# naver/dust3r

Hardware: NVIDIA H100
Metric: image-pairs/sec (512x384, ViT-L/B+DPT) (higher is better)
Workload: dtype bf16

## Files before the change

dust3r_b200/_lib_fwd.py:

```python
import ctypes as C

F_BIAS, F_GELU, F_RELU, F_OUT_F32, F_RESID_INPLACE = 1, 2, 4, 8, 16
F_ADD0, F_ADD1, F_OUT2_RELU, F_ROPE, F_OUT2_BF16 = 32, 64, 128, 256, 2048


class Linear(C.Structure):
    _fields_ = [('w', C.c_void_p), ('b', C.c_void_p)]


class Norm(C.Structure):
    _fields_ = [('g', C.c_void_p), ('b', C.c_void_p)]


class EncBlock(C.Structure):
    _fields_ = [('norm1', Norm), ('norm2', Norm), ('qkv', Linear), ('proj', Linear), ('fc1', Linear), ('fc2', Linear)]


class DecBlock(C.Structure):
    _fields_ = [('norm1', Norm), ('norm2', Norm), ('norm3', Norm), ('norm_y', Norm),
                ('qkv', Linear), ('proj', Linear), ('projq', Linear), ('projkv', Linear), ('cproj', Linear),
                ('fc1', Linear), ('fc2', Linear)]


class Fusion(C.Structure):
    _fields_ = [('rcu1_conv1', Linear), ('rcu1_conv2', Linear), ('rcu2_conv1', Linear), ('rcu2_conv2', Linear),
                ('out_conv', Linear)]


class DptHead(C.Structure):
    _fields_ = [('act_conv', Linear * 4), ('act0_up', Linear), ('act1_up', Linear), ('act3_down', Linear),
                ('layer_rn', Linear * 4), ('refine', Fusion * 4), ('head0', Linear), ('head2', Linear),
                ('head4_w', C.c_void_p), ('head4_b', C.c_void_p)]


class Model(C.Structure):
    _fields_ = [('enc_dim', C.c_int32), ('enc_depth', C.c_int32), ('enc_heads', C.c_int32), ('dec_dim', C.c_int32),
                ('dec_depth', C.c_int32), ('dec_heads', C.c_int32), ('mlp_ratio', C.c_int32), ('patch', C.c_int32),
                ('head_type', C.c_int32), ('nch', C.c_int32), ('depth_mode', C.c_int32), ('conf_mode', C.c_int32),
                ('conf_min', C.c_float), ('conf_max', C.c_float), ('ln_eps', C.c_float),
                ('hooks', C.c_int32 * 4), ('rope_max_pos', C.c_int32),
                ('rope_cos', C.c_void_p), ('rope_sin', C.c_void_p),
                ('patch_embed', Linear), ('enc', C.POINTER(EncBlock)), ('enc_norm', Norm), ('decoder_embed', Linear),
                ('dec1', C.POINTER(DecBlock)), ('dec2', C.POINTER(DecBlock)), ('dec_norm', Norm),
                ('dpt', C.POINTER(DptHead) * 2), ('lin_head', Linear * 2)]


def declare(lib):
    vp, i32, i64, u32, f32 = C.c_void_p, C.c_int32, C.c_int64, C.c_uint32, C.c_float
    lib.d3r_gemm_bf16.restype = C.c_int
    lib.d3r_gemm_bf16.argtypes = [vp, vp, vp, vp, vp, vp, i32, i32, i32, i64, u32, vp, vp, i32, i32, i32, vp]
    lib.d3r_conv3x3_bf16.restype = C.c_int
    lib.d3r_conv3x3_bf16.argtypes = [vp, vp, vp, vp, vp, vp, vp, i32, i32, i32, i32, i32, u32, vp]
    lib.d3r_attention_hd64.restype = C.c_int
    lib.d3r_attention_hd64.argtypes = [vp, i64, vp, i64, vp, i64, vp, i64, i32, i32, i32, i32, f32, vp]
    lib.d3r_conv_transpose_bf16.restype = C.c_int
    lib.d3r_conv_transpose_bf16.argtypes = [vp, vp, vp, vp, i32, i32, i32, i32, i32, i32, vp]
    lib.d3r_conv3x3_head_tail.restype = C.c_int
    lib.d3r_conv3x3_head_tail.argtypes = [vp, vp, vp, vp, vp, vp, vp, i32, i32, i32, i32, i32, f32, f32, vp]
    lib.d3r_layernorm_bf16.restype = C.c_int
    lib.d3r_layernorm_bf16.argtypes = [vp, vp, vp, vp, i32, i32, f32, vp]
    lib.d3r_upsample2x_bf16.restype = C.c_int
    lib.d3r_upsample2x_bf16.argtypes = [vp, vp, i32, i32, i32, i32, i32, i32, vp]
    lib.d3r_im2col_3x3_s2_bf16.restype = C.c_int
    lib.d3r_im2col_3x3_s2_bf16.argtypes = [vp, vp, i32, i32, i32, i32, vp]
    lib.d3r_patch_im2col16.restype = C.c_int
    lib.d3r_patch_im2col16.argtypes = [vp, vp, i32, i32, i32, vp]
    lib.d3r_linear_head_postprocess.restype = C.c_int
    lib.d3r_linear_head_postprocess.argtypes = [vp, vp, vp, i32, i32, i32, i32, i32, i32, f32, f32, vp]
    lib.d3r_set_gemm_impl.restype = None
    lib.d3r_set_gemm_impl.argtypes = [i32]
    lib.d3r_set_gemm_store.restype = None
    lib.d3r_set_gemm_store.argtypes = [i32]
    lib.d3r_set_attention_impl.restype = None
    lib.d3r_set_attention_impl.argtypes = [i32]
    lib.d3r_forward_workspace_bytes.restype = i64
    lib.d3r_forward_workspace_bytes.argtypes = [C.POINTER(Model), i32, i32, i32, i32]
    lib.d3r_forward_pairs.restype = C.c_int
    lib.d3r_forward_pairs.argtypes = [C.POINTER(Model), vp, i32, C.POINTER(i32), C.POINTER(i32), i32, i32, i32,
                                      vp, vp, vp, vp, vp, i64, vp]
    lib.d3r_forward_mixed_workspace_bytes.restype = i64
    lib.d3r_forward_mixed_workspace_bytes.argtypes = [C.POINTER(Model), i32, i32, i32, i32, i32]
    lib.d3r_forward_pairs_mixed.restype = C.c_int
    lib.d3r_forward_pairs_mixed.argtypes = [C.POINTER(Model), vp, i32, i32, vp, i32, i32, i32, vp, vp, vp, vp, vp, i64, vp]
    lib.d3r_forward_set_debug.restype = C.c_int
    lib.d3r_forward_set_debug.argtypes = [i32, vp, i64]
    lib.d3r_sizeof_model.restype = C.c_int
```

dust3r_b200/csrc/gemm_host.cu:

```cuda
#include "gemm_wgmma.cuh"
#include "gemm_host.h"
#include "prof.h"

namespace d3r {
namespace gemm {

static int pick_block_n(int N, int mode, uint32_t flags) {
  if (flags & F_HEAD_FINAL) return 128;
  if (N % 256 == 0 && pick_epi(mode, flags) != EPI_GENERIC) return 256;
  if (N % 128 == 0) return 128;
  if (N % 64 == 0) return 64;
  return (N > 128) ? 128 : 64;
}

static int g_impl = 2;
static int g_pair_min_kb = 4;
static bool use_pair(int bn, int num_kb) { return bn >= 128 && (g_impl == 1 || (g_impl == 2 && num_kb >= g_pair_min_kb)); }

static int g_store = 1;

template <int BN, int EPI, bool PAIR, bool TMA_STORE = false>
static int launch(const CUtensorMap& ta, const CUtensorMap& tb, const CUtensorMap& to, const Params& p, int m_tiles, int n_tiles,
                  cudaStream_t st) {
  constexpr int kSmem = Cfg<BN, TMA_STORE>::kSmemBytes;
  static unsigned long long attr_devices = 0;
  if (first_launch_on_this_device(attr_devices))
    D3R_CUDA(cudaFuncSetAttribute(gemm_kernel<BN, EPI, PAIR, TMA_STORE>, cudaFuncAttributeMaxDynamicSharedMemorySize, kSmem));
  int grid;
  if (PAIR) {
    const int items = ((m_tiles + 1) / 2) * n_tiles;
    const int max_clusters = num_sms() / 2;
    grid = 2 * (items < max_clusters ? items : max_clusters);
  } else {
    const int items = m_tiles * n_tiles;
    grid = items < num_sms() ? items : num_sms();
  }
  const char* tag = (p.mode == 1) ? ((p.flags & F_HEAD_FINAL) ? (PAIR ? "conv3x3_head_tail_2cta" : "conv3x3_head_tail")
                                                              : (PAIR ? "conv3x3_wgmma_2cta" : "conv3x3_wgmma"))
                                  : (BN == 256 ? (PAIR ? "gemm_wgmma_2cta_bn256" : "gemm_wgmma_bn256")
                                               : (PAIR ? "gemm_wgmma_2cta_bn128" : (BN == 128 ? "gemm_wgmma_bn128" : "gemm_wgmma_bn64")));
  char detail[96];
  snprintf(detail, sizeof(detail), "M=%d N=%d K=%d flags=0x%x mode=%d epi=%d", p.M, p.N, p.K, (unsigned)p.flags, p.mode, EPI);
  prof::Scope scope(tag, st, 2.0 * double(p.M) * double(p.N) * double(p.K), 0.0, 1, detail);
  D3R_CUDA(pdl::launch_clustered(gemm_kernel<BN, EPI, PAIR, TMA_STORE>, dim3(grid), dim3(kNumThreads), size_t(kSmem), st, PAIR ? 2 : 1,
                                 ta, tb, to, p));
  D3R_LAUNCH_CHECK();
  return D3R_OK;
}

template <int BN, bool PAIR>
static int dispatch_epi(int epi, const CUtensorMap& ta, const CUtensorMap& tb, const CUtensorMap* to, const Params& p, int m_tiles,
                        int n_tiles, cudaStream_t st) {
  if constexpr (BN == 256) {
    if (to) {
      switch (epi) {
        case EPI_RESID: return launch<BN, EPI_RESID, PAIR, true>(ta, tb, *to, p, m_tiles, n_tiles, st);
        case EPI_ACT: return launch<BN, EPI_ACT, PAIR, true>(ta, tb, *to, p, m_tiles, n_tiles, st);
        case EPI_ROPE: return launch<BN, EPI_ROPE, PAIR, true>(ta, tb, *to, p, m_tiles, n_tiles, st);
      }
    }
  }
  switch (epi) {
    case EPI_RESID: return launch<BN, EPI_RESID, PAIR>(ta, tb, tb, p, m_tiles, n_tiles, st);
    case EPI_ACT: return launch<BN, EPI_ACT, PAIR>(ta, tb, tb, p, m_tiles, n_tiles, st);
    case EPI_ROPE: return launch<BN, EPI_ROPE, PAIR>(ta, tb, tb, p, m_tiles, n_tiles, st);
  }
  if constexpr (BN == 128) return launch<128, EPI_GENERIC, PAIR>(ta, tb, tb, p, m_tiles, n_tiles, st);
  set_error("no BLOCK_N %d kernel for the generic epilogue", BN);
  return D3R_ERR_INVALID;
}

static int dispatch(int bn, const CUtensorMap& ta, const CUtensorMap& tb, const CUtensorMap* to, const Params& p, int m_tiles,
                    cudaStream_t st) {
  const int n_tiles = (p.N + bn - 1) / bn;
  const int epi = (bn >= 128) ? pick_epi(p.mode, p.flags) : EPI_GENERIC;
  const bool pair = use_pair(bn, p.num_kb);
  switch (bn) {
    case 256: return pair ? dispatch_epi<256, true>(epi, ta, tb, to, p, m_tiles, n_tiles, st) : dispatch_epi<256, false>(epi, ta, tb, to, p, m_tiles, n_tiles, st);
    case 128: return pair ? dispatch_epi<128, true>(epi, ta, tb, nullptr, p, m_tiles, n_tiles, st) : dispatch_epi<128, false>(epi, ta, tb, nullptr, p, m_tiles, n_tiles, st);
    case 64: return launch<64, EPI_GENERIC, false>(ta, tb, tb, p, m_tiles, n_tiles, st);
  }
  set_error("unsupported BLOCK_N %d", bn);
  return D3R_ERR_INVALID;
}

static int make_tmap_b(CUtensorMap* m, const void* B, int N, int taps, int Kc, int bn, int num_kb, const char* op) {
  cuuint64_t dims[3] = {(cuuint64_t)Kc, (cuuint64_t)taps, (cuuint64_t)N};
  cuuint64_t str[2] = {(cuuint64_t)Kc * 2, (cuuint64_t)taps * Kc * 2};
  cuuint32_t box[3] = {(cuuint32_t)BLOCK_K, 1, (cuuint32_t)(use_pair(bn, num_kb) ? bn / 2 : bn)};
  return encode_tensor_map(m, B, 3, dims, str, box, op);
}

int gemm_bf16(const void* A, long long lda, const void* B, Params p, cudaStream_t st) {
  D3R_CHECK_ARG(A && B, "gemm: null operand");
  D3R_CHECK_ARG(p.M > 0 && p.N > 0 && p.K > 0, "gemm: bad shape %d %d %d", p.M, p.N, p.K);
  D3R_CHECK_ARG(p.N % 32 == 0, "gemm: N=%d must be a multiple of 32", p.N);
  D3R_CHECK_ARG(p.K % 8 == 0 && lda % 8 == 0, "gemm: K=%d / lda=%lld must be multiples of 8 (16-byte TMA strides)", p.K, lda);
  D3R_CHECK_ARG((reinterpret_cast<uintptr_t>(A) & 15) == 0 && (reinterpret_cast<uintptr_t>(B) & 15) == 0, "gemm: operands must be 16-byte aligned");
  p.mode = 0;
  p.num_kb = (p.K + BLOCK_K - 1) / BLOCK_K;
  const int bn = pick_block_n(p.N, p.mode, p.flags);
  CUtensorMap ta, tb;
  {
    cuuint64_t dims[2] = {(cuuint64_t)p.K, (cuuint64_t)p.M};
    cuuint64_t str[1] = {(cuuint64_t)lda * 2};
    cuuint32_t box[2] = {(cuuint32_t)BLOCK_K, (cuuint32_t)BLOCK_M};
    int rc = encode_tensor_map(&ta, A, 2, dims, str, box, "gemm");
    if (rc) return rc;
  }
  int rc = make_tmap_b(&tb, B, p.N, 1, p.K, bn, p.num_kb, "gemm");
  if (rc) return rc;
  CUtensorMap to;
  const bool f32 = (p.flags & F_RESID_INPLACE) != 0;
  const long long row_bytes = p.ldo * (f32 ? 4 : 2);
  const bool staged = g_store == 1 && bn == 256 && pick_epi(p.mode, p.flags) != EPI_GENERIC && p.ldo >= p.N && row_bytes % 16 == 0 &&
                      (reinterpret_cast<uintptr_t>(p.out) & 15) == 0;
  if (staged) {
    cuuint64_t dims[2] = {(cuuint64_t)p.N, (cuuint64_t)p.M};
    cuuint64_t str[1] = {(cuuint64_t)row_bytes};
    cuuint32_t box[2] = {(cuuint32_t)(f32 ? 32 : 64), 64};
    rc = encode_tensor_map(&to, p.out, 2, dims, str, box, "gemm output", f32 ? CU_TENSOR_MAP_DATA_TYPE_FLOAT32 : CU_TENSOR_MAP_DATA_TYPE_BFLOAT16);
    if (rc) return rc;
  }
  return dispatch(bn, ta, tb, staged ? &to : nullptr, p, (p.M + BLOCK_M - 1) / BLOCK_M, st);
}

int conv3x3_bf16(const void* x_nhwc, const void* w_packed, int B, int H, int W, int Cin, int Cout, Params p, cudaStream_t st) {
  D3R_CHECK_ARG(x_nhwc && w_packed, "conv3x3: null operand");
  D3R_CHECK_ARG(Cin % 8 == 0 && Cout % 32 == 0, "conv3x3: Cin=%d must be a multiple of 8 and Cout=%d of 32", Cin, Cout);
  p.mode = 1;
  p.M = B * H * W;
  p.N = Cout;
  p.cin_blocks = (Cin + BLOCK_K - 1) / BLOCK_K;
  p.K = 9 * Cin;
  p.num_kb = 9 * p.cin_blocks;
  p.cB = B; p.cH = H; p.cW = W;
  int tw = 16;
  while (tw < W && tw < 128) tw *= 2;
  p.tile_w = tw;
  p.tile_h = BLOCK_M / tw;
  p.tiles_x = (W + p.tile_w - 1) / p.tile_w;
  p.tiles_y = (H + p.tile_h - 1) / p.tile_h;
  p.ldo = Cout;
  const int bn = pick_block_n(p.N, p.mode, p.flags);
  CUtensorMap ta, tb;
  {
    cuuint64_t dims[4] = {(cuuint64_t)Cin, (cuuint64_t)W, (cuuint64_t)H, (cuuint64_t)B};
    cuuint64_t str[3] = {(cuuint64_t)Cin * 2, (cuuint64_t)W * Cin * 2, (cuuint64_t)H * W * Cin * 2};
    cuuint32_t box[4] = {(cuuint32_t)BLOCK_K, (cuuint32_t)p.tile_w, (cuuint32_t)p.tile_h, 1};
    int rc = encode_tensor_map(&ta, x_nhwc, 4, dims, str, box, "conv3x3");
    if (rc) return rc;
  }
  int rc = make_tmap_b(&tb, w_packed, Cout, 9, Cin, bn, p.num_kb, "conv3x3");
  if (rc) return rc;
  return dispatch(bn, ta, tb, nullptr, p, B * p.tiles_x * p.tiles_y, st);
}

int conv_transpose_bf16(const void* x_nhwc, const void* w_packed, void* out, const float* bias, int B, int h, int w, int Cin, int Cout,
                        int k, cudaStream_t st) {
  D3R_CHECK_ARG(x_nhwc && w_packed && out, "conv_transpose: null buffer");
  D3R_CHECK_ARG(B > 0 && h > 0 && w > 0 && Cin > 0 && Cout > 0 && k > 0, "conv_transpose: bad shape B=%d h=%d w=%d Cin=%d Cout=%d k=%d", B,
                h, w, Cin, Cout, k);
  D3R_CHECK_ARG(Cin % 8 == 0, "conv_transpose: Cin=%d must be a multiple of 8", Cin);
  D3R_CHECK_ARG(Cout % 2 == 0 && (k * k * Cout) % 32 == 0, "conv_transpose: Cout=%d must be even and k*k*Cout=%d a multiple of 32", Cout,
                k * k * Cout);
  Params p{};
  p.M = B * h * w; p.N = k * k * Cout; p.K = Cin;
  p.flags = F_CONVT | (bias ? F_BIAS : 0);
  p.out = out; p.bias = bias; p.ldo = 0;
  p.tk = k; p.th_in = h; p.tw_in = w; p.tCout = Cout;
  return gemm_bf16(x_nhwc, Cin, w_packed, p, st);
}

int conv3x3_head_tail(const void* x_nhwc, const void* w_packed, const float* bias, const float* w4, const float* b4, float* pts3d,
                      float* conf, int B, int H, int W, int depth_mode, int conf_mode, float conf_min, float conf_max, cudaStream_t st) {
  D3R_CHECK_ARG(x_nhwc && w_packed && w4 && b4 && pts3d, "conv3x3_head_tail: null buffer");
  D3R_CHECK_ARG(B > 0 && H > 0 && W > 0, "conv3x3_head_tail: bad shape B=%d H=%d W=%d", B, H, W);
  D3R_CHECK_ARG(depth_mode >= 0 && depth_mode <= 2, "conv3x3_head_tail: depth_mode %d out of range", depth_mode);
  D3R_CHECK_ARG(conf_mode >= 0 && conf_mode <= 2, "conv3x3_head_tail: conf_mode %d out of range", conf_mode);
  D3R_CHECK_ARG(conf_mode == 0 || conf, "conv3x3_head_tail: conf_mode %d without a conf buffer", conf_mode);
  Params p{};
  p.flags = F_HEAD_FINAL | (bias ? F_BIAS : 0);
  p.bias = bias;
  p.w4 = w4; p.b4 = b4;
  p.pts3d = pts3d; p.conf = conf;
  p.depth_mode = depth_mode; p.conf_mode = conf_mode;
  p.conf_min = conf_min; p.conf_max = conf_max;
  return conv3x3_bf16(x_nhwc, w_packed, B, H, W, 128, 128, p, st);
}

}
}

using namespace d3r;

extern "C" void d3r_set_gemm_impl(int32_t impl) { gemm::g_impl = impl; }
extern "C" void d3r_set_gemm_pair_min_kblocks(int32_t kb) { gemm::g_pair_min_kb = kb; }
extern "C" void d3r_set_gemm_store(int32_t store) { gemm::g_store = store; }

extern "C" int d3r_gemm_bf16(const void* A, const void* B, void* out, const float* bias, const void* add0, void* out2,
                             int32_t M, int32_t N, int32_t K, int64_t ldo, uint32_t flags, const float* rope_cos,
                             const float* rope_sin, int32_t rope_cols, int32_t tokens_per_img, int32_t grid_w, void* stream) {
  gemm::Params p{};
  p.M = M; p.N = N; p.K = K;
  p.flags = flags;
  p.out = out; p.out2 = out2; p.add0 = add0; p.bias = bias; p.ldo = ldo;
  p.rope_cos = rope_cos; p.rope_sin = rope_sin; p.rope_cols = rope_cols; p.tokens_per_img = tokens_per_img; p.grid_w = grid_w;
  D3R_CHECK_ARG(!(flags & gemm::F_BIAS) || bias, "gemm: F_BIAS without bias");
  D3R_CHECK_ARG(!(flags & gemm::F_ROPE) || (rope_cos && rope_sin && tokens_per_img > 0 && grid_w > 0), "gemm: F_ROPE without tables");
  D3R_CHECK_ARG(!(flags & (gemm::F_CONVT | gemm::F_HEAD_FINAL)),
                "gemm: F_CONVT / F_HEAD_FINAL have their own entry points, d3r_conv_transpose_bf16 / d3r_conv3x3_head_tail");
  return gemm::gemm_bf16(A, K, B, p, (cudaStream_t)stream);
}

extern "C" int d3r_conv3x3_bf16(const void* x_nhwc, const void* w_packed, void* out, const float* bias, const void* add0,
                                const void* add1, void* out2, int32_t B, int32_t H, int32_t W, int32_t Cin, int32_t Cout,
                                uint32_t flags, void* stream) {
  gemm::Params p{};
  p.flags = flags;
  p.out = out; p.out2 = out2; p.add0 = add0; p.add1 = add1; p.bias = bias;
  D3R_CHECK_ARG(!(flags & (gemm::F_CONVT | gemm::F_HEAD_FINAL | gemm::F_ROPE)), "conv3x3: unsupported flag");
  return gemm::conv3x3_bf16(x_nhwc, w_packed, B, H, W, Cin, Cout, p, (cudaStream_t)stream);
}

extern "C" int d3r_conv_transpose_bf16(const void* x_nhwc, const void* w_packed, void* out, const float* bias, int32_t B, int32_t h,
                                       int32_t w, int32_t Cin, int32_t Cout, int32_t k, void* stream) {
  return gemm::conv_transpose_bf16(x_nhwc, w_packed, out, bias, B, h, w, Cin, Cout, k, (cudaStream_t)stream);
}

extern "C" int d3r_conv3x3_head_tail(const void* x_nhwc, const void* w_packed, const float* bias, const float* w4, const float* b4,
                                     float* pts3d, float* conf, int32_t B, int32_t H, int32_t W, int32_t depth_mode, int32_t conf_mode,
                                     float conf_min, float conf_max, void* stream) {
  return gemm::conv3x3_head_tail(x_nhwc, w_packed, bias, w4, b4, pts3d, conf, B, H, W, depth_mode, conf_mode, conf_min, conf_max,
                                 (cudaStream_t)stream);
}
```

dust3r_b200/csrc/gemm_wgmma.cuh:

```cuda
#pragma once
#include "d3r_common.cuh"
#include "sm90_ptx.cuh"
#include "pdl.cuh"

namespace d3r {
namespace gemm {

constexpr int BLOCK_M = 128;
constexpr int BLOCK_K = 64;
constexpr int WGMMA_K = 16;
constexpr int kNumThreads = 384;
constexpr int kConsumerWarps = 8;

enum : uint32_t {
  F_BIAS = 1u << 0,
  F_GELU = 1u << 1,
  F_RELU = 1u << 2,
  F_OUT_F32 = 1u << 3,
  F_RESID_INPLACE = 1u << 4,
  F_ADD0 = 1u << 5,
  F_ADD1 = 1u << 6,
  F_OUT2_RELU = 1u << 7,
  F_ROPE = 1u << 8,
  F_CONVT = 1u << 9,
  F_HEAD_FINAL = 1u << 10,
  F_OUT2_BF16 = 1u << 11,
};

struct Params {
  int M, N, K;
  int num_kb;
  int mode;
  uint32_t flags;
  void* out;
  void* out2;
  const void* add0;
  const void* add1;
  const float* bias;
  long long ldo;
  const float* rope_cos;
  const float* rope_sin;
  int rope_cols, tokens_per_img, grid_w;
  int cB, cH, cW, cin_blocks, tile_w, tile_h, tiles_x, tiles_y;
  int tk, th_in, tw_in, tCout;
  const float* w4;
  const float* b4;
  float* pts3d;
  float* conf;
  int depth_mode;
  int conf_mode;
  float conf_min, conf_max;
};

enum : int { EPI_GENERIC = 0, EPI_RESID = 1, EPI_ACT = 2, EPI_ROPE = 3 };
template <int EPI> struct EpiMask { static constexpr uint32_t value = 0xFFFFFFFFu; };
template <> struct EpiMask<EPI_RESID> { static constexpr uint32_t value = F_BIAS | F_RESID_INPLACE; };
template <> struct EpiMask<EPI_ACT> { static constexpr uint32_t value = F_BIAS | F_GELU | F_RELU; };
template <> struct EpiMask<EPI_ROPE> { static constexpr uint32_t value = F_BIAS | F_ROPE; };
__host__ __device__ inline int pick_epi(int mode, uint32_t flags) {
  if (mode != 0) return EPI_GENERIC;
  if ((flags & ~F_BIAS) == F_RESID_INPLACE) return EPI_RESID;
  if ((flags & ~EpiMask<EPI_ACT>::value) == 0) return EPI_ACT;
  if ((flags & ~EpiMask<EPI_ROPE>::value) == 0) return EPI_ROPE;
  return EPI_GENERIC;
}

template <int BLOCK_N, bool TMA_STORE = false>
struct Cfg {
  static constexpr int kStageA = BLOCK_M * BLOCK_K * 2;
  static constexpr int kStageB = BLOCK_N * BLOCK_K * 2;
  static constexpr int kStages = (BLOCK_N == 256) ? 4 : (BLOCK_N == 128) ? 6 : 8;
  static constexpr int kRing = kStages * (kStageA + kStageB);
  static constexpr int kOutBuf = 64 * 128;
  static constexpr int kStaging = TMA_STORE ? 2 * 2 * kOutBuf : 0;
  static constexpr int kSmemBytes = kRing + kStaging + 1024  + 256  + (TMA_STORE ? 0 : (4 * 128 + 16) * 4) ;
  static_assert(kSmemBytes <= 227 * 1024, "shared memory of one CTA");
};

__device__ __forceinline__ float gelu_erf(float x) {
  constexpr float kU = 0.84932180028801904f;
  constexpr float kP = 0.3275911f * 0.70710678118654752f / kU;
  const float u = fabsf(x) * kU;
  const float t = ptx::rcp_approx(fmaf(kP, u, 1.f));
  float poly = fmaf(0.5f * 1.061405429f, t, 0.5f * -1.453152027f);
  poly = fmaf(poly, t, 0.5f * 1.421413741f);
  poly = fmaf(poly, t, 0.5f * -0.284496736f);
  poly = fmaf(poly, t, 0.5f * 0.254829592f);
  const float e = ptx::ex2_approx(-u * u);
  const float h = x * (poly * t * e);
  return fmaxf(x, 0.f) - fabsf(h);
}

template <int BLOCK_N, int EPI, bool PAIR, bool TMA_STORE>
__global__ void __launch_bounds__(kNumThreads, 1)
gemm_kernel(const __grid_constant__ CUtensorMap tmap_a, const __grid_constant__ CUtensorMap tmap_b,
            const __grid_constant__ CUtensorMap tmap_o, const Params p) {
  static_assert(!TMA_STORE || (BLOCK_N == 256 && EPI != EPI_GENERIC), "TMA-store epilogue: specialised epilogues on 128x256 tiles");
  using C = Cfg<BLOCK_N, TMA_STORE>;
  extern __shared__ uint8_t smem_raw[];
  uint8_t* smem = reinterpret_cast<uint8_t*>((reinterpret_cast<uintptr_t>(smem_raw) + 1023) & ~uintptr_t(1023));
  uint8_t* smem_a = smem;
  uint8_t* smem_b = smem + C::kStages * C::kStageA;
  uint8_t* smem_o = smem + C::kRing;
  uint64_t* bars = reinterpret_cast<uint64_t*>(smem + C::kRing + C::kStaging);
  uint64_t* full_bar = bars;
  uint64_t* empty_bar = bars + C::kStages;
  float* s_w4 = reinterpret_cast<float*>(reinterpret_cast<uint8_t*>(bars) + 256);

  const int warp = threadIdx.x >> 5, lane = threadIdx.x & 31;
  const uint32_t rank = PAIR ? ptx::cluster_ctarank() : 0u;
  const int n_tiles = (p.N + BLOCK_N - 1) / BLOCK_N;
  const int m_tiles = (p.mode == 1) ? p.cB * p.tiles_y * p.tiles_x : (p.M + BLOCK_M - 1) / BLOCK_M;
  const int m_groups = PAIR ? (m_tiles + 1) / 2 : m_tiles;
  const int total_items = m_groups * n_tiles;
  const int first_item = PAIR ? blockIdx.x / 2 : blockIdx.x;
  const int item_stride = PAIR ? gridDim.x / 2 : gridDim.x;

  if (threadIdx.x == 0) {
    ptx::prefetch_tmap(&tmap_a);
    ptx::prefetch_tmap(&tmap_b);
    if constexpr (TMA_STORE) ptx::prefetch_tmap(&tmap_o);
    for (int s = 0; s < C::kStages; ++s) {
      ptx::mbar_init(ptx::smem_u32(&full_bar[s]), 1);
      ptx::mbar_init(ptx::smem_u32(&empty_bar[s]), (PAIR ? 2 : 1) * kConsumerWarps);
    }
    ptx::fence_barrier_init();
  }
  if (!TMA_STORE && (p.flags & F_HEAD_FINAL) && threadIdx.x >= 128) {
    for (int i = threadIdx.x - 128; i < 4 * 128 + 4; i += 256) s_w4[i] = (i < 512) ? p.w4[i] : p.b4[i - 512];
  }
  __syncthreads();
  if constexpr (PAIR) ptx::cluster_sync();
  pdl::sync_with_predecessor();

  if (warp < 4) {
    ptx::setmaxnreg_dec<40>();
    if (warp == 0 && ptx::elect_one()) {
      int stage = 0;
      uint32_t phase = 0;
      for (int item = first_item; item < total_items; item += item_stride) {
        const int tn = item % n_tiles, tm = (item / n_tiles) * (PAIR ? 2 : 1) + int(rank);
        int cb = 0, cy0 = 0, cx0 = 0;
        if (p.mode == 1) {
          cb = tm / (p.tiles_y * p.tiles_x);
          const int r = tm - cb * (p.tiles_y * p.tiles_x);
          cy0 = (r / p.tiles_x) * p.tile_h;
          cx0 = (r % p.tiles_x) * p.tile_w;
        }
        for (int kb = 0; kb < p.num_kb; ++kb) {
          ptx::mbar_wait(ptx::smem_u32(&empty_bar[stage]), phase ^ 1);
          const uint32_t fb = ptx::smem_u32(&full_bar[stage]);
          ptx::mbar_arrive_expect_tx(fb, C::kStageA + C::kStageB);
          const uint32_t sa = ptx::smem_u32(smem_a + stage * C::kStageA);
          const uint32_t sb = ptx::smem_u32(smem_b + stage * C::kStageB);
          int ka, kt = 0;
          if (p.mode == 1) {
            const int tap = kb / p.cin_blocks, cblk = kb - tap * p.cin_blocks;
            const int dy = tap / 3, dx = tap - dy * 3;
            ptx::tma_load_4d(sa, &tmap_a, fb, cblk * BLOCK_K, cx0 + dx - 1, cy0 + dy - 1, cb);
            ka = cblk * BLOCK_K;
            kt = tap;
          } else {
            ptx::tma_load_2d(sa, &tmap_a, fb, kb * BLOCK_K, tm * BLOCK_M);
            ka = kb * BLOCK_K;
          }
          if constexpr (PAIR) {
            constexpr int kHalf = BLOCK_N / 2;
            ptx::tma_load_3d_mc(sb + rank * (kHalf * BLOCK_K * 2), &tmap_b, fb, ka, kt, tn * BLOCK_N + int(rank) * kHalf, 0x3);
          } else {
            ptx::tma_load_3d(sb, &tmap_b, fb, ka, kt, tn * BLOCK_N);
          }
          if (++stage == C::kStages) { stage = 0; phase ^= 1; }
        }
      }
    }
  } else {
    ptx::setmaxnreg_inc<232>();
    const int wg = (threadIdx.x >> 7) - 1;
    const int wq = warp & 3;
    const int q = lane & 3;
    const uint32_t flags = p.flags & EpiMask<EPI>::value;
    constexpr int kNB = BLOCK_N / 8;
    float acc[BLOCK_N / 2];
    int stage = 0;
    uint32_t phase = 0;
    uint32_t out_chunk = 0;
    auto release = [&](int s) {
      if (lane == 0) {
        if constexpr (PAIR) {
          ptx::mbar_arrive_cluster(ptx::smem_u32(&empty_bar[s]), 0);
          ptx::mbar_arrive_cluster(ptx::smem_u32(&empty_bar[s]), 1);
        } else {
          ptx::mbar_arrive(ptx::smem_u32(&empty_bar[s]));
        }
      }
    };
    for (int item = first_item; item < total_items; item += item_stride) {
      const int tn = item % n_tiles, tm = (item / n_tiles) * (PAIR ? 2 : 1) + int(rank);
      int prev = -1;
      for (int kb = 0; kb < p.num_kb; ++kb) {
        ptx::mbar_wait(ptx::smem_u32(&full_bar[stage]), phase);
        const uint64_t da = ptx::desc_kmajor_sw128(ptx::smem_u32(smem_a + stage * C::kStageA + wg * 64 * 128));
        const uint64_t db = ptx::desc_kmajor_sw128(ptx::smem_u32(smem_b + stage * C::kStageB));
        ptx::wgmma_fence();
#pragma unroll
        for (int k = 0; k < BLOCK_K / WGMMA_K; ++k) {
          if constexpr (BLOCK_N == 256) ptx::wgmma_m64n256k16_ss(acc, da + uint64_t(2 * k), db + uint64_t(2 * k), (kb | k) != 0 ? 1u : 0u);
          else if constexpr (BLOCK_N == 128) ptx::wgmma_m64n128k16_ss(acc, da + uint64_t(2 * k), db + uint64_t(2 * k), (kb | k) != 0 ? 1u : 0u);
          else ptx::wgmma_m64n64k16_ss(acc, da + uint64_t(2 * k), db + uint64_t(2 * k), (kb | k) != 0 ? 1u : 0u);
        }
        ptx::wgmma_commit();
        ptx::wgmma_wait<1>();
        if (prev >= 0) release(prev);
        prev = stage;
        if (++stage == C::kStages) { stage = 0; phase ^= 1; }
      }
      ptx::wgmma_wait<0>();
      ptx::reg_fence(acc);
      release(prev);

      bool valid[2];
      long long row_off[2];
      int tok[2] = {0, 0};
      long long pix[2] = {0, 0};
      int ct_b[2] = {0, 0}, ct_iy[2] = {0, 0}, ct_ix[2] = {0, 0};
#pragma unroll
      for (int h = 0; h < 2; ++h) {
        const int row_in_tile = wg * 64 + wq * 16 + (lane >> 2) + 8 * h;
        if (p.mode == 1) {
          const int cb = tm / (p.tiles_y * p.tiles_x);
          const int r = tm - cb * (p.tiles_y * p.tiles_x);
          const int y = (r / p.tiles_x) * p.tile_h + row_in_tile / p.tile_w;
          const int x = (r % p.tiles_x) * p.tile_w + row_in_tile % p.tile_w;
          valid[h] = (tm < m_tiles) && (y < p.cH) && (x < p.cW);
          pix[h] = (long long)(cb * p.cH + y) * p.cW + x;
          row_off[h] = pix[h] * p.ldo;
        } else {
          const int row = tm * BLOCK_M + row_in_tile;
          valid[h] = row < p.M;
          row_off[h] = (long long)row * p.ldo;
          if (flags & F_ROPE) tok[h] = row % p.tokens_per_img;
          if (flags & F_CONVT) {
            ct_b[h] = row / (p.th_in * p.tw_in);
            const int r = row - ct_b[h] * (p.th_in * p.tw_in);
            ct_iy[h] = r / p.tw_in;
            ct_ix[h] = r - ct_iy[h] * p.tw_in;
          }
        }
      }
      if (flags & (F_BIAS | F_GELU)) {
#pragma unroll
        for (int j = 0; j < kNB; ++j) {
          const int c = tn * BLOCK_N + 8 * j + 2 * q;
          float2 b = make_float2(0.f, 0.f);
          if ((flags & F_BIAS) && c < p.N) {
            if (flags & F_CONVT) b = make_float2(__ldg(p.bias + c % p.tCout), __ldg(p.bias + (c + 1) % p.tCout));
            else b = __ldg(reinterpret_cast<const float2*>(p.bias + c));
          }
#pragma unroll
          for (int h = 0; h < 2; ++h) {
            float& v0 = acc[4 * j + 2 * h];
            float& v1 = acc[4 * j + 2 * h + 1];
            v0 += b.x;
            v1 += b.y;
            if (flags & F_GELU) { v0 = gelu_erf(v0); v1 = gelu_erf(v1); }
          }
        }
      }
      if (flags & F_ROPE) {
#pragma unroll
        for (int cb = 0; cb < BLOCK_N / 32; ++cb) {
          const int col0 = tn * BLOCK_N + cb * 32;
          if (col0 >= p.rope_cols) continue;
#pragma unroll
          for (int h = 0; h < 2; ++h) {
            const int pos = ((col0 & 63) < 32) ? (tok[h] / p.grid_w) : (tok[h] % p.grid_w);
#pragma unroll
            for (int jj = 0; jj < 2; ++jj) {
              const int k = 8 * jj + 2 * q;
              const float2 cs = __ldg(reinterpret_cast<const float2*>(p.rope_cos + pos * 16 + k));
              const float2 sn = __ldg(reinterpret_cast<const float2*>(p.rope_sin + pos * 16 + k));
              const float cc[2] = {cs.x, cs.y}, ss[2] = {sn.x, sn.y};
#pragma unroll
              for (int e = 0; e < 2; ++e) {
                float& u = acc[(4 * cb + jj) * 4 + 2 * h + e];
                float& w = acc[(4 * cb + jj + 2) * 4 + 2 * h + e];
                const float u0 = u, w0 = w;
                u = u0 * cc[e] - w0 * ss[e];
                w = w0 * cc[e] + u0 * ss[e];
              }
            }
          }
        }
      }
      if constexpr (TMA_STORE) {
        constexpr bool kF32 = (EPI == EPI_RESID);
        constexpr int kChunkCols = kF32 ? 32 : 64;
        constexpr int kChunkNB = kChunkCols / 8;
        const bool issuer = (threadIdx.x & 127) == 0;
        const uint32_t sw = lane >> 2;
#pragma unroll
        for (int c = 0; c < BLOCK_N / kChunkCols; ++c) {
          const uint32_t buf = ptx::smem_u32(smem_o + (wg * 2 + (out_chunk & 1)) * C::kOutBuf);
#pragma unroll
          for (int j = 0; j < kChunkNB; ++j)
#pragma unroll
            for (int h = 0; h < 2; ++h) {
              const uint32_t row = wq * 16 + (lane >> 2) + 8 * h;
              float v0 = acc[4 * (c * kChunkNB + j) + 2 * h], v1 = acc[4 * (c * kChunkNB + j) + 2 * h + 1];
              if (flags & F_RELU) { v0 = fmaxf(v0, 0.f); v1 = fmaxf(v1, 0.f); }
              if constexpr (kF32) {
                ptx::st_shared_v2_f32(buf + row * 128 + (((2 * j + (q >> 1)) ^ sw) << 4) + (q & 1) * 8, v0, v1);
              } else {
                ptx::st_shared_b32(buf + row * 128 + ((j ^ sw) << 4) + q * 4, pack_bf16x2(v0, v1));
              }
            }
          ptx::fence_proxy_async();
          if (issuer) ptx::bulk_wait_group_read<0>();
          ptx::named_bar_sync(1 + wg, 128);
          if (issuer) {
            const int c0 = tn * BLOCK_N + c * kChunkCols, r0 = tm * BLOCK_M + wg * 64;
            if constexpr (kF32) ptx::tma_reduce_add_2d(&tmap_o, buf, c0, r0);
            else ptx::tma_store_2d(&tmap_o, buf, c0, r0);
            ptx::bulk_commit_group();
          }
          ++out_chunk;
        }
        continue;
      }
      if (flags & F_HEAD_FINAL) {
        float head_acc[2][4] = {{0.f, 0.f, 0.f, 0.f}, {0.f, 0.f, 0.f, 0.f}};
#pragma unroll
        for (int j = 0; j < kNB; ++j)
#pragma unroll
          for (int h = 0; h < 2; ++h)
#pragma unroll
            for (int e = 0; e < 2; ++e) {
              const float r = fmaxf(acc[4 * j + 2 * h + e], 0.f);
              const int c = 8 * j + 2 * q + e;
#pragma unroll
              for (int o = 0; o < 4; ++o) head_acc[h][o] += r * s_w4[o * 128 + c];
            }
#pragma unroll
        for (int h = 0; h < 2; ++h)
#pragma unroll
          for (int o = 0; o < 4; ++o) {
            head_acc[h][o] += __shfl_xor_sync(0xffffffffu, head_acc[h][o], 1);
            head_acc[h][o] += __shfl_xor_sync(0xffffffffu, head_acc[h][o], 2);
          }
#pragma unroll
        for (int h = 0; h < 2; ++h) {
          if (!valid[h] || q != 0) continue;
          postprocess_pixel(head_acc[h][0] + s_w4[512 + 0], head_acc[h][1] + s_w4[512 + 1], head_acc[h][2] + s_w4[512 + 2],
                            [&] { return head_acc[h][3] + s_w4[512 + 3]; }, p.pts3d, p.conf, pix[h], p.depth_mode, p.conf_mode,
                            p.conf_min, p.conf_max);
        }
        continue;
      }
#pragma unroll
      for (int h = 0; h < 2; ++h) {
        if (!valid[h]) continue;
#pragma unroll
        for (int j = 0; j < kNB; ++j) {
          const int col = tn * BLOCK_N + 8 * j + 2 * q;
          if (col >= p.N) continue;
          float v0 = acc[4 * j + 2 * h], v1 = acc[4 * j + 2 * h + 1];
          long long off;
          if (flags & F_CONVT) {
            const int kk = col / p.tCout, co = col - kk * p.tCout;
            const int ky = kk / p.tk, kx = kk - ky * p.tk;
            off = ((long long)(ct_b[h] * p.th_in * p.tk + ct_iy[h] * p.tk + ky) * (p.tw_in * p.tk) + ct_ix[h] * p.tk + kx) * p.tCout + co;
          } else {
            off = row_off[h] + col;
          }
          if (flags & F_ADD0) {
            const float2 a = bf16x2_to_float2(__ldg(reinterpret_cast<const unsigned int*>(reinterpret_cast<const __nv_bfloat16*>(p.add0) + off)));
            v0 += a.x; v1 += a.y;
          }
          if (flags & F_ADD1) {
            const float2 a = bf16x2_to_float2(__ldg(reinterpret_cast<const unsigned int*>(reinterpret_cast<const __nv_bfloat16*>(p.add1) + off)));
            v0 += a.x; v1 += a.y;
          }
          if (flags & F_RELU) { v0 = fmaxf(v0, 0.f); v1 = fmaxf(v1, 0.f); }
          if (flags & (F_OUT_F32 | F_RESID_INPLACE)) {
            float2* o = reinterpret_cast<float2*>(reinterpret_cast<float*>(p.out) + off);
            if (flags & F_RESID_INPLACE) {
              const float2 r = *o;
              v0 += r.x; v1 += r.y;
            }
            *o = make_float2(v0, v1);
            if (flags & F_OUT2_BF16) *reinterpret_cast<uint32_t*>(reinterpret_cast<__nv_bfloat16*>(p.out2) + off) = pack_bf16x2(v0, v1);
          } else {
            *reinterpret_cast<uint32_t*>(reinterpret_cast<__nv_bfloat16*>(p.out) + off) = pack_bf16x2(v0, v1);
            if (flags & F_OUT2_RELU)
              *reinterpret_cast<uint32_t*>(reinterpret_cast<__nv_bfloat16*>(p.out2) + off) = pack_bf16x2(fmaxf(v0, 0.f), fmaxf(v1, 0.f));
          }
        }
      }
    }
    if constexpr (TMA_STORE) {
      if ((threadIdx.x & 127) == 0) ptx::bulk_wait_group<0>();
    }
  }
  if constexpr (PAIR) ptx::cluster_sync();
}

}
}
```

dust3r_b200/csrc/sm90_ptx.cuh:

```cuda
#pragma once
#include <cuda.h>
#include <cuda_runtime.h>
#include <cuda_bf16.h>
#include <cstdint>

namespace d3r {
namespace ptx {

__device__ __forceinline__ uint32_t smem_u32(const void* p) { return static_cast<uint32_t>(__cvta_generic_to_shared(p)); }

__device__ __forceinline__ bool elect_one() {
  uint32_t pred = 0;
  asm volatile(
      "{\n"
      ".reg .b32 %%rx;\n"
      ".reg .pred %%px;\n"
      "elect.sync %%rx|%%px, %1;\n"
      "@%%px mov.s32 %0, 1;\n"
      "}\n"
      : "+r"(pred)
      : "r"(0xffffffffu));
  return pred != 0;
}

__device__ __forceinline__ void mbar_init(uint32_t bar, uint32_t count) {
  asm volatile("mbarrier.init.shared::cta.b64 [%0], %1;" ::"r"(bar), "r"(count));
}
__device__ __forceinline__ void fence_barrier_init() { asm volatile("fence.mbarrier_init.release.cluster;" ::: "memory"); }
__device__ __forceinline__ void fence_proxy_async() { asm volatile("fence.proxy.async.shared::cta;" ::: "memory"); }

__device__ __forceinline__ void mbar_arrive_expect_tx(uint32_t bar, uint32_t bytes) {
  asm volatile("mbarrier.arrive.expect_tx.shared::cta.b64 _, [%0], %1;" ::"r"(bar), "r"(bytes) : "memory");
}
__device__ __forceinline__ void mbar_arrive(uint32_t bar) {
  asm volatile("mbarrier.arrive.shared::cta.b64 _, [%0];" ::"r"(bar) : "memory");
}
__device__ __forceinline__ bool mbar_try_wait(uint32_t bar, uint32_t parity) {
  uint32_t done;
  asm volatile(
      "{\n"
      ".reg .pred p;\n"
      "mbarrier.try_wait.parity.shared::cta.b64 p, [%1], %2;\n"
      "selp.u32 %0, 1, 0, p;\n"
      "}\n"
      : "=r"(done)
      : "r"(bar), "r"(parity)
      : "memory");
  return done != 0;
}
__device__ __forceinline__ void mbar_wait(uint32_t bar, uint32_t parity) {
  while (!mbar_try_wait(bar, parity)) {
  }
}
__device__ __forceinline__ void mbar_wait_bounded(uint32_t bar, uint32_t parity) {
  uint32_t spins = 0;
  bool done;
  do {
    done = mbar_try_wait(bar, parity);
    if (!done && ++spins > (1u << 22)) __trap();
  } while (!done);
}

__device__ __forceinline__ void bulk_g2s(uint32_t dst, const void* src, uint32_t bytes, uint32_t bar) {
  asm volatile("cp.async.bulk.shared::cluster.global.mbarrier::complete_tx::bytes [%0], [%1], %2, [%3];"
               ::"r"(dst), "l"(src), "r"(bytes), "r"(bar) : "memory");
}
__device__ __forceinline__ uint64_t policy_evict_first() {
  uint64_t pol;
  asm volatile("createpolicy.fractional.L2::evict_first.b64 %0, 1.0;" : "=l"(pol));
  return pol;
}
__device__ __forceinline__ void bulk_g2s_hint(uint32_t dst, const void* src, uint32_t bytes, uint32_t bar, uint64_t pol) {
  asm volatile("cp.async.bulk.shared::cluster.global.mbarrier::complete_tx::bytes.L2::cache_hint [%0], [%1], %2, [%3], %4;"
               ::"r"(dst), "l"(src), "r"(bytes), "r"(bar), "l"(pol) : "memory");
}

__device__ __forceinline__ void prefetch_tmap(const void* tmap) {
  asm volatile("prefetch.tensormap [%0];" ::"l"(reinterpret_cast<uint64_t>(tmap)) : "memory");
}
__device__ __forceinline__ void tma_load_2d(uint32_t dst, const void* tmap, uint32_t bar, int c0, int c1) {
  asm volatile(
      "cp.async.bulk.tensor.2d.shared::cluster.global.mbarrier::complete_tx::bytes [%0], [%1, {%3, %4}], [%2];"
      ::"r"(dst), "l"(reinterpret_cast<uint64_t>(tmap)), "r"(bar), "r"(c0), "r"(c1)
      : "memory");
}
__device__ __forceinline__ void tma_load_3d(uint32_t dst, const void* tmap, uint32_t bar, int c0, int c1, int c2) {
  asm volatile(
      "cp.async.bulk.tensor.3d.shared::cluster.global.mbarrier::complete_tx::bytes [%0], [%1, {%3, %4, %5}], [%2];"
      ::"r"(dst), "l"(reinterpret_cast<uint64_t>(tmap)), "r"(bar), "r"(c0), "r"(c1), "r"(c2)
      : "memory");
}
__device__ __forceinline__ void tma_load_4d(uint32_t dst, const void* tmap, uint32_t bar, int c0, int c1, int c2, int c3) {
  asm volatile(
      "cp.async.bulk.tensor.4d.shared::cluster.global.mbarrier::complete_tx::bytes [%0], [%1, {%3, %4, %5, %6}], [%2];"
      ::"r"(dst), "l"(reinterpret_cast<uint64_t>(tmap)), "r"(bar), "r"(c0), "r"(c1), "r"(c2), "r"(c3)
      : "memory");
}
__device__ __forceinline__ void tma_load_3d_mc(uint32_t dst, const void* tmap, uint32_t bar, int c0, int c1, int c2, uint16_t mask) {
  asm volatile(
      "cp.async.bulk.tensor.3d.shared::cluster.global.mbarrier::complete_tx::bytes.multicast::cluster [%0], [%1, {%3, %4, %5}], [%2], %6;"
      ::"r"(dst), "l"(reinterpret_cast<uint64_t>(tmap)), "r"(bar), "r"(c0), "r"(c1), "r"(c2), "h"(mask)
      : "memory");
}

__device__ __forceinline__ void tma_store_2d(const void* tmap, uint32_t src, int c0, int c1) {
  asm volatile("cp.async.bulk.tensor.2d.global.shared::cta.tile.bulk_group [%0, {%2, %3}], [%1];"
               ::"l"(reinterpret_cast<uint64_t>(tmap)), "r"(src), "r"(c0), "r"(c1) : "memory");
}
__device__ __forceinline__ void tma_reduce_add_2d(const void* tmap, uint32_t src, int c0, int c1) {
  asm volatile("cp.reduce.async.bulk.tensor.2d.global.shared::cta.add.tile.bulk_group [%0, {%2, %3}], [%1];"
               ::"l"(reinterpret_cast<uint64_t>(tmap)), "r"(src), "r"(c0), "r"(c1) : "memory");
}
__device__ __forceinline__ void bulk_commit_group() { asm volatile("cp.async.bulk.commit_group;" ::: "memory"); }
template <int N> __device__ __forceinline__ void bulk_wait_group_read() { asm volatile("cp.async.bulk.wait_group.read %0;" ::"n"(N) : "memory"); }
template <int N> __device__ __forceinline__ void bulk_wait_group() { asm volatile("cp.async.bulk.wait_group %0;" ::"n"(N) : "memory"); }
__device__ __forceinline__ void st_shared_b32(uint32_t addr, uint32_t v) { asm volatile("st.shared.b32 [%0], %1;" ::"r"(addr), "r"(v) : "memory"); }
__device__ __forceinline__ void st_shared_v2_f32(uint32_t addr, float a, float b) {
  asm volatile("st.shared.v2.f32 [%0], {%1, %2};" ::"r"(addr), "f"(a), "f"(b) : "memory");
}
__device__ __forceinline__ void named_bar_sync(uint32_t id, uint32_t count) { asm volatile("bar.sync %0, %1;" ::"r"(id), "r"(count) : "memory"); }

__device__ __forceinline__ uint32_t cluster_ctarank() {
  uint32_t r;
  asm volatile("mov.u32 %0, %%cluster_ctarank;" : "=r"(r));
  return r;
}
__device__ __forceinline__ void cluster_sync() {
  asm volatile("barrier.cluster.arrive.release.aligned;\nbarrier.cluster.wait.acquire.aligned;" ::: "memory");
}
__device__ __forceinline__ void mbar_arrive_cluster(uint32_t bar, uint32_t rank) {
  asm volatile(
      "{\n"
      ".reg .b32 raddr;\n"
      "mapa.shared::cluster.u32 raddr, %0, %1;\n"
      "mbarrier.arrive.shared::cluster.b64 _, [raddr];\n"
      "}\n" ::"r"(bar), "r"(rank) : "memory");
}

__device__ __forceinline__ float ex2_approx(float x) { float y; asm("ex2.approx.ftz.f32 %0, %1;" : "=f"(y) : "f"(x)); return y; }
__device__ __forceinline__ float rcp_approx(float x) { float y; asm("rcp.approx.ftz.f32 %0, %1;" : "=f"(y) : "f"(x)); return y; }
__device__ __forceinline__ float rsqrt_approx(float x) { float y; asm("rsqrt.approx.ftz.f32 %0, %1;" : "=f"(y) : "f"(x)); return y; }
__device__ __forceinline__ float sqrt_approx(float x) { float y; asm("sqrt.approx.ftz.f32 %0, %1;" : "=f"(y) : "f"(x)); return y; }

template <int N> __device__ __forceinline__ void setmaxnreg_dec() { asm volatile("setmaxnreg.dec.sync.aligned.u32 %0;" ::"n"(N)); }
template <int N> __device__ __forceinline__ void setmaxnreg_inc() { asm volatile("setmaxnreg.inc.sync.aligned.u32 %0;" ::"n"(N)); }

__device__ __forceinline__ void wgmma_fence() { asm volatile("wgmma.fence.sync.aligned;" ::: "memory"); }
__device__ __forceinline__ void wgmma_commit() { asm volatile("wgmma.commit_group.sync.aligned;" ::: "memory"); }
template <int N> __device__ __forceinline__ void wgmma_wait() { asm volatile("wgmma.wait_group.sync.aligned %0;" ::"n"(N) : "memory"); }
template <int N> __device__ __forceinline__ void reg_fence(float (&d)[N]) {
#pragma unroll
  for (int i = 0; i < N; ++i) asm volatile("" : "+f"(d[i])::"memory");
}

__device__ __forceinline__ uint64_t desc_sw128(uint32_t smem_addr, uint32_t lbo_bytes) {
  uint64_t d = 0;
  d |= uint64_t((smem_addr & 0x3FFFF) >> 4);
  d |= uint64_t(lbo_bytes >> 4) << 16;
  d |= uint64_t(1024 >> 4) << 32;
  d |= uint64_t(1) << 62;
  return d;
}
__device__ __forceinline__ uint64_t desc_kmajor_sw128(uint32_t smem_addr) { return desc_sw128(smem_addr, 16); }
__device__ __forceinline__ uint64_t desc_mnmajor_sw128(uint32_t smem_addr) { return desc_sw128(smem_addr, 1024); }

__device__ __forceinline__ void wgmma_m64n64k16_ss(float* d, uint64_t desc_a, uint64_t desc_b, uint32_t accumulate) {
  asm volatile(
      "{\n"
      ".reg .pred p;\n"
      "setp.ne.b32 p, %34, 0;\n"
      "wgmma.mma_async.sync.aligned.m64n64k16.f32.bf16.bf16 "
      "{%0, %1, %2, %3, %4, %5, %6, %7, %8, %9, %10, %11, %12, %13, %14, %15, %16, %17, %18, %19, %20, %21, %22, %23, %24, %25, %26, %27, %28, %29, %30, %31}, %32, %33, p, 1, 1, 0, 0;\n"
      "}\n"
      : "+f"(d[0]), "+f"(d[1]), "+f"(d[2]), "+f"(d[3]), "+f"(d[4]), "+f"(d[5]), "+f"(d[6]), "+f"(d[7]), "+f"(d[8]), "+f"(d[9]), "+f"(d[10]), "+f"(d[11]), "+f"(d[12]), "+f"(d[13]), "+f"(d[14]), "+f"(d[15]), "+f"(d[16]), "+f"(d[17]), "+f"(d[18]), "+f"(d[19]), "+f"(d[20]), "+f"(d[21]), "+f"(d[22]), "+f"(d[23]), "+f"(d[24]), "+f"(d[25]), "+f"(d[26]), "+f"(d[27]), "+f"(d[28]), "+f"(d[29]), "+f"(d[30]), "+f"(d[31])
      : "l"(desc_a), "l"(desc_b), "r"(accumulate));
}
__device__ __forceinline__ void wgmma_m64n128k16_ss(float* d, uint64_t desc_a, uint64_t desc_b, uint32_t accumulate) {
  asm volatile(
      "{\n"
      ".reg .pred p;\n"
      "setp.ne.b32 p, %66, 0;\n"
      "wgmma.mma_async.sync.aligned.m64n128k16.f32.bf16.bf16 "
      "{%0, %1, %2, %3, %4, %5, %6, %7, %8, %9, %10, %11, %12, %13, %14, %15, %16, %17, %18, %19, %20, %21, %22, %23, %24, %25, %26, %27, %28, %29, %30, %31, %32, %33, %34, %35, %36, %37, %38, %39, %40, %41, %42, %43, %44, %45, %46, %47, %48, %49, %50, %51, %52, %53, %54, %55, %56, %57, %58, %59, %60, %61, %62, %63}, %64, %65, p, 1, 1, 0, 0;\n"
      "}\n"
      : "+f"(d[0]), "+f"(d[1]), "+f"(d[2]), "+f"(d[3]), "+f"(d[4]), "+f"(d[5]), "+f"(d[6]), "+f"(d[7]), "+f"(d[8]), "+f"(d[9]), "+f"(d[10]), "+f"(d[11]), "+f"(d[12]), "+f"(d[13]), "+f"(d[14]), "+f"(d[15]), "+f"(d[16]), "+f"(d[17]), "+f"(d[18]), "+f"(d[19]), "+f"(d[20]), "+f"(d[21]), "+f"(d[22]), "+f"(d[23]), "+f"(d[24]), "+f"(d[25]), "+f"(d[26]), "+f"(d[27]), "+f"(d[28]), "+f"(d[29]), "+f"(d[30]), "+f"(d[31]), "+f"(d[32]), "+f"(d[33]), "+f"(d[34]), "+f"(d[35]), "+f"(d[36]), "+f"(d[37]), "+f"(d[38]), "+f"(d[39]), "+f"(d[40]), "+f"(d[41]), "+f"(d[42]), "+f"(d[43]), "+f"(d[44]), "+f"(d[45]), "+f"(d[46]), "+f"(d[47]), "+f"(d[48]), "+f"(d[49]), "+f"(d[50]), "+f"(d[51]), "+f"(d[52]), "+f"(d[53]), "+f"(d[54]), "+f"(d[55]), "+f"(d[56]), "+f"(d[57]), "+f"(d[58]), "+f"(d[59]), "+f"(d[60]), "+f"(d[61]), "+f"(d[62]), "+f"(d[63])
      : "l"(desc_a), "l"(desc_b), "r"(accumulate));
}
__device__ __forceinline__ void wgmma_m64n256k16_ss(float* d, uint64_t desc_a, uint64_t desc_b, uint32_t accumulate) {
  asm volatile(
      "{\n"
      ".reg .pred p;\n"
      "setp.ne.b32 p, %130, 0;\n"
      "wgmma.mma_async.sync.aligned.m64n256k16.f32.bf16.bf16 "
      "{%0, %1, %2, %3, %4, %5, %6, %7, %8, %9, %10, %11, %12, %13, %14, %15, %16, %17, %18, %19, %20, %21, %22, %23, %24, %25, %26, %27, %28, %29, %30, %31, %32, %33, %34, %35, %36, %37, %38, %39, %40, %41, %42, %43, %44, %45, %46, %47, %48, %49, %50, %51, %52, %53, %54, %55, %56, %57, %58, %59, %60, %61, %62, %63, %64, %65, %66, %67, %68, %69, %70, %71, %72, %73, %74, %75, %76, %77, %78, %79, %80, %81, %82, %83, %84, %85, %86, %87, %88, %89, %90, %91, %92, %93, %94, %95, %96, %97, %98, %99, %100, %101, %102, %103, %104, %105, %106, %107, %108, %109, %110, %111, %112, %113, %114, %115, %116, %117, %118, %119, %120, %121, %122, %123, %124, %125, %126, %127}, %128, %129, p, 1, 1, 0, 0;\n"
      "}\n"
      : "+f"(d[0]), "+f"(d[1]), "+f"(d[2]), "+f"(d[3]), "+f"(d[4]), "+f"(d[5]), "+f"(d[6]), "+f"(d[7]), "+f"(d[8]), "+f"(d[9]), "+f"(d[10]), "+f"(d[11]), "+f"(d[12]), "+f"(d[13]), "+f"(d[14]), "+f"(d[15]), "+f"(d[16]), "+f"(d[17]), "+f"(d[18]), "+f"(d[19]), "+f"(d[20]), "+f"(d[21]), "+f"(d[22]), "+f"(d[23]), "+f"(d[24]), "+f"(d[25]), "+f"(d[26]), "+f"(d[27]), "+f"(d[28]), "+f"(d[29]), "+f"(d[30]), "+f"(d[31]), "+f"(d[32]), "+f"(d[33]), "+f"(d[34]), "+f"(d[35]), "+f"(d[36]), "+f"(d[37]), "+f"(d[38]), "+f"(d[39]), "+f"(d[40]), "+f"(d[41]), "+f"(d[42]), "+f"(d[43]), "+f"(d[44]), "+f"(d[45]), "+f"(d[46]), "+f"(d[47]), "+f"(d[48]), "+f"(d[49]), "+f"(d[50]), "+f"(d[51]), "+f"(d[52]), "+f"(d[53]), "+f"(d[54]), "+f"(d[55]), "+f"(d[56]), "+f"(d[57]), "+f"(d[58]), "+f"(d[59]), "+f"(d[60]), "+f"(d[61]), "+f"(d[62]), "+f"(d[63]), "+f"(d[64]), "+f"(d[65]), "+f"(d[66]), "+f"(d[67]), "+f"(d[68]), "+f"(d[69]), "+f"(d[70]), "+f"(d[71]), "+f"(d[72]), "+f"(d[73]), "+f"(d[74]), "+f"(d[75]), "+f"(d[76]), "+f"(d[77]), "+f"(d[78]), "+f"(d[79]), "+f"(d[80]), "+f"(d[81]), "+f"(d[82]), "+f"(d[83]), "+f"(d[84]), "+f"(d[85]), "+f"(d[86]), "+f"(d[87]), "+f"(d[88]), "+f"(d[89]), "+f"(d[90]), "+f"(d[91]), "+f"(d[92]), "+f"(d[93]), "+f"(d[94]), "+f"(d[95]), "+f"(d[96]), "+f"(d[97]), "+f"(d[98]), "+f"(d[99]), "+f"(d[100]), "+f"(d[101]), "+f"(d[102]), "+f"(d[103]), "+f"(d[104]), "+f"(d[105]), "+f"(d[106]), "+f"(d[107]), "+f"(d[108]), "+f"(d[109]), "+f"(d[110]), "+f"(d[111]), "+f"(d[112]), "+f"(d[113]), "+f"(d[114]), "+f"(d[115]), "+f"(d[116]), "+f"(d[117]), "+f"(d[118]), "+f"(d[119]), "+f"(d[120]), "+f"(d[121]), "+f"(d[122]), "+f"(d[123]), "+f"(d[124]), "+f"(d[125]), "+f"(d[126]), "+f"(d[127])
      : "l"(desc_a), "l"(desc_b), "r"(accumulate));
}
__device__ __forceinline__ void wgmma_m64n64k16_rs_tb(float* d, const uint32_t* a, uint64_t desc_b, uint32_t accumulate) {
  asm volatile(
      "{\n"
      ".reg .pred p;\n"
      "setp.ne.b32 p, %37, 0;\n"
      "wgmma.mma_async.sync.aligned.m64n64k16.f32.bf16.bf16 "
      "{%0, %1, %2, %3, %4, %5, %6, %7, %8, %9, %10, %11, %12, %13, %14, %15, %16, %17, %18, %19, %20, %21, %22, %23, %24, %25, %26, %27, %28, %29, %30, %31}, {%32, %33, %34, %35}, %36, p, 1, 1, 1;\n"
      "}\n"
      : "+f"(d[0]), "+f"(d[1]), "+f"(d[2]), "+f"(d[3]), "+f"(d[4]), "+f"(d[5]), "+f"(d[6]), "+f"(d[7]), "+f"(d[8]), "+f"(d[9]), "+f"(d[10]), "+f"(d[11]), "+f"(d[12]), "+f"(d[13]), "+f"(d[14]), "+f"(d[15]), "+f"(d[16]), "+f"(d[17]), "+f"(d[18]), "+f"(d[19]), "+f"(d[20]), "+f"(d[21]), "+f"(d[22]), "+f"(d[23]), "+f"(d[24]), "+f"(d[25]), "+f"(d[26]), "+f"(d[27]), "+f"(d[28]), "+f"(d[29]), "+f"(d[30]), "+f"(d[31])
      : "r"(a[0]), "r"(a[1]), "r"(a[2]), "r"(a[3]), "l"(desc_b), "r"(accumulate));
}
__device__ __forceinline__ void wgmma_m64n64k16_ss_tb(float* d, uint64_t desc_a, uint64_t desc_b, uint32_t accumulate) {
  asm volatile(
      "{\n"
      ".reg .pred p;\n"
      "setp.ne.b32 p, %34, 0;\n"
      "wgmma.mma_async.sync.aligned.m64n64k16.f32.bf16.bf16 "
      "{%0, %1, %2, %3, %4, %5, %6, %7, %8, %9, %10, %11, %12, %13, %14, %15, %16, %17, %18, %19, %20, %21, %22, %23, %24, %25, %26, %27, %28, %29, %30, %31}, %32, %33, p, 1, 1, 0, 1;\n"
      "}\n"
      : "+f"(d[0]), "+f"(d[1]), "+f"(d[2]), "+f"(d[3]), "+f"(d[4]), "+f"(d[5]), "+f"(d[6]), "+f"(d[7]), "+f"(d[8]), "+f"(d[9]), "+f"(d[10]), "+f"(d[11]), "+f"(d[12]), "+f"(d[13]), "+f"(d[14]), "+f"(d[15]), "+f"(d[16]), "+f"(d[17]), "+f"(d[18]), "+f"(d[19]), "+f"(d[20]), "+f"(d[21]), "+f"(d[22]), "+f"(d[23]), "+f"(d[24]), "+f"(d[25]), "+f"(d[26]), "+f"(d[27]), "+f"(d[28]), "+f"(d[29]), "+f"(d[30]), "+f"(d[31])
      : "l"(desc_a), "l"(desc_b), "r"(accumulate));
}

}
}
```

include/dust3r_b200.h:

```cpp
#ifndef DUST3R_B200_H_
#define DUST3R_B200_H_

#include <stddef.h>
#include <stdint.h>

#ifdef __cplusplus
extern "C" {
#endif

#define D3R_OK 0
#define D3R_ERR_INVALID (-1)
#define D3R_ERR_CUDA (-2)
#define D3R_ERR_UNSUPPORTED_DEVICE (-3)

const char* d3r_last_error(void);
int d3r_abi_version(void);
int d3r_check_device(void);

long long d3r_launch_count(void);
void d3r_launch_count_reset(void);
void d3r_prof_enable(int on);
int d3r_prof_report(char* buf, int cap);
int d3r_prof_dump(char* buf, int cap);


typedef struct d3r_align_desc {
  int32_t n_imgs;
  int32_t n_edges;
  int32_t n_entries;
  int32_t n_chunks;
  int32_t max_deg;
  int32_t max_chunks;
  int32_t chunk_px;
  int32_t dist_l2;
  int32_t norm_pw_scale;
  int32_t tied_focal;
  int32_t eval_only;
  float base_scale;
  float pw_break;
  float focal_break;
  float adam_eps;
  float beta1, beta2;

  const int32_t* img_hw;
  const int64_t* img_pix_off;
  const int32_t* img_ent_ptr;
  const int32_t* img_chunk_ptr;
  const int32_t* chunk_img;
  const int32_t* ent_edge;
  const int64_t* ent_obs_off;
  const float*   ent_coef;
  const int32_t* edge_ent;
  const void* obs;

  float* logd;
  float* logd_m;
  float* logd_v;
  float* small;
  float* small_m;
  float* small_v;
  const uint8_t* small_trainable;

  float* workspace;
  const float* sched;
  float* loss_out;
  int32_t* counters;

  int32_t stream_kernel;
  int32_t stream_grid;
  int32_t stream_ppt;
  int32_t stream_window;
  int32_t n_items;
  int32_t reserved0;
  const void* items;
  const int32_t* warp_item_ptr;
  const void* items_rev;
  const int32_t* warp_item_ptr_rev;
} d3r_align_desc;

typedef struct d3r_align_item {
  int32_t img, slot0, nslots, npx;
  int32_t e0, deg, W, u0;
  int32_t v0;
  float inv_w;
  int64_t pix0;
  int64_t obs0;
  int32_t slab_units;
  int32_t reserved;
} d3r_align_item;

int d3r_sizeof_align_desc(void);
int d3r_sizeof_align_item(void);
int d3r_align_chunk_pixels(void);
int64_t d3r_align_workspace_floats(int32_t n_imgs, int32_t n_edges);
int d3r_align_prepare(const d3r_align_desc* desc, void* stream);
int d3r_align_run(const d3r_align_desc* desc, int32_t it_begin, int32_t it_end, void* stream);
int d3r_align_loss_grad(const d3r_align_desc* desc, float* logd_grad, float* small_grad, float* entry_loss, void* stream);
int d3r_align_overflow_flag(const d3r_align_desc* desc, int32_t* host_out, void* stream);
int d3r_align_pts3d(const d3r_align_desc* desc, float* out_dev, void* stream);
int d3r_align_set_debug(void* dev_buf);

#define D3R_CONF_ID 0
#define D3R_CONF_LOG 1
#define D3R_CONF_SQRT 2
#define D3R_CONF_M1 3
typedef struct d3r_pack_entry {
  const float* pts;
  const float* conf;
  int64_t obs_off;
  int32_t area;
  float coef;
} d3r_pack_entry;
int d3r_sizeof_pack_entry(void);
int d3r_align_stream_slots_per_item(void);
int d3r_align_stream_warps_per_cta(void);
int d3r_align_stream_max_window(void);
int d3r_align_pack_entries(const d3r_pack_entry* table_dev, int32_t n_entries, int32_t max_area, int32_t conf_mode,
                           int32_t stream_layout, void* obs_dev, void* stream);


#define D3R_F_BIAS          (1u << 0)
#define D3R_F_GELU          (1u << 1)
#define D3R_F_RELU          (1u << 2)
#define D3R_F_OUT_F32       (1u << 3)
#define D3R_F_RESID_INPLACE (1u << 4)
#define D3R_F_ADD0          (1u << 5)
#define D3R_F_ADD1          (1u << 6)
#define D3R_F_OUT2_RELU     (1u << 7)
#define D3R_F_ROPE          (1u << 8)
#define D3R_F_OUT2_BF16     (1u << 11)

int d3r_gemm_bf16(const void* A_dev, const void* B_dev, void* out_dev, const float* bias_dev, const void* add0_dev,
                  void* out2_dev, int32_t M, int32_t N, int32_t K, int64_t ldo, uint32_t flags,
                  const float* rope_cos_dev, const float* rope_sin_dev, int32_t rope_cols, int32_t tokens_per_img,
                  int32_t grid_w, void* stream);

int d3r_conv3x3_bf16(const void* x_nhwc_dev, const void* w_packed_dev, void* out_dev, const float* bias_dev,
                     const void* add0_dev, const void* add1_dev, void* out2_dev, int32_t B, int32_t H, int32_t W,
                     int32_t Cin, int32_t Cout, uint32_t flags, void* stream);

int d3r_attention_hd64(const void* q_dev, int64_t ldq, const void* k_dev, int64_t ldk, const void* v_dev, int64_t ldv,
                       void* out_dev, int64_t ldo, int32_t B, int32_t heads, int32_t Nq, int32_t Nk, float scale,
                       void* stream);

int d3r_conv_transpose_bf16(const void* x_nhwc_dev, const void* w_packed_dev, void* out_dev, const float* bias_dev, int32_t B,
                            int32_t h, int32_t w, int32_t Cin, int32_t Cout, int32_t k, void* stream);

int d3r_conv3x3_head_tail(const void* x_nhwc_dev, const void* w_packed_dev, const float* bias_dev, const float* w4_dev,
                          const float* b4_dev, float* pts3d_dev, float* conf_dev, int32_t B, int32_t H, int32_t W, int32_t depth_mode,
                          int32_t conf_mode, float conf_min, float conf_max, void* stream);

int d3r_layernorm_bf16(const float* x_dev, const float* g_dev, const float* b_dev, void* out_dev, int32_t M, int32_t C, float eps,
                       void* stream);

int d3r_upsample2x_bf16(const void* x_dev, void* out_dev, int32_t B, int32_t H, int32_t W, int32_t C, int32_t Ho, int32_t Wo,
                        void* stream);

int d3r_im2col_3x3_s2_bf16(const void* x_dev, void* out_dev, int32_t B, int32_t H, int32_t W, int32_t C, void* stream);

int d3r_patch_im2col16(const float* img_dev, void* out_dev, int32_t B, int32_t H, int32_t W, void* stream);

int d3r_linear_head_postprocess(const float* feat_dev, float* pts3d_dev, float* conf_dev, int32_t B, int32_t gh, int32_t gw,
                                int32_t nch, int32_t depth_mode, int32_t conf_mode, float conf_min, float conf_max, void* stream);

void d3r_set_gemm_impl(int32_t impl);
void d3r_set_gemm_pair_min_kblocks(int32_t kblocks);
void d3r_set_gemm_store(int32_t store);

void d3r_set_attention_impl(int32_t impl);

int d3r_clean_pointcloud(int32_t n_imgs, const int32_t* hw_dev, const int64_t* off_dev, int32_t max_area, const float* pts3d_dev,
                         float* conf_dev, const float* depth_dev, const float* K_dev, const float* cams_dev, float tol,
                         float bad_conf, void* stream);
int d3r_procrustes_moments(int32_t n_problems, int32_t n_points, const float* x_dev, const float* y_dev, const float* w_dev,
                           double* out_dev, void* stream);
int d3r_weiszfeld_focal(int32_t n_maps, int32_t H, int32_t W, const float* pts3d_dev, const float* pp_dev, int32_t steps,
                        float* focal_dev, void* stream);
int d3r_nearest_neighbours(int32_t n_queries, int32_t n_points, const float* queries_dev, const float* points_dev, int32_t* nn_dev,
                           void* stream);
int d3r_image_resize_crop_normalize(const uint8_t* src_dev, int32_t H0, int32_t W0, int32_t H1, int32_t W1,
                                    const int32_t* xbounds_dev, const int32_t* xcoefs_dev, int32_t kx,
                                    const int32_t* ybounds_dev, const int32_t* ycoefs_dev, int32_t ky, int32_t row0, int32_t rows,
                                    int32_t crop_x0, int32_t crop_y0, int32_t H2, int32_t W2, const float* lut_dev, uint8_t* tmp_dev,
                                    float* out_dev, void* stream);
int64_t d3r_segment_sky_workspace_bytes(int32_t n_imgs, int64_t total_px);
int d3r_segment_sky(int32_t n_imgs, const int32_t* hw_dev, const int64_t* off_dev, int32_t max_area, int64_t total_px,
                    const uint8_t* rgb_dev, uint8_t* sky_out_dev, void* workspace_dev, int64_t workspace_bytes, void* stream);

typedef struct d3r_linear { const void* w; const float* b; } d3r_linear;
typedef struct d3r_norm { const float* g; const float* b; } d3r_norm;

typedef struct d3r_enc_block {
  d3r_norm norm1, norm2;
  d3r_linear qkv, proj, fc1, fc2;
} d3r_enc_block;

typedef struct d3r_dec_block {
  d3r_norm norm1, norm2, norm3, norm_y;
  d3r_linear qkv, proj;
  d3r_linear projq, projkv, cproj;
  d3r_linear fc1, fc2;
} d3r_dec_block;

typedef struct d3r_fusion {
  d3r_linear rcu1_conv1, rcu1_conv2, rcu2_conv1, rcu2_conv2;
  d3r_linear out_conv;
} d3r_fusion;

typedef struct d3r_dpt_head {
  d3r_linear act_conv[4];
  d3r_linear act0_up;
  d3r_linear act1_up;
  d3r_linear act3_down;
  d3r_linear layer_rn[4];
  d3r_fusion refine[4];
  d3r_linear head0;
  d3r_linear head2;
  const float* head4_w;
  const float* head4_b;
} d3r_dpt_head;

typedef struct d3r_model {
  int32_t enc_dim, enc_depth, enc_heads, dec_dim, dec_depth, dec_heads, mlp_ratio, patch;
  int32_t head_type;
  int32_t nch;
  int32_t depth_mode;
  int32_t conf_mode;
  float conf_min, conf_max, ln_eps;
  int32_t hooks[4];
  int32_t rope_max_pos;
  const float* rope_cos;
  const float* rope_sin;
  d3r_linear patch_embed;
  const d3r_enc_block* enc;
  d3r_norm enc_norm;
  d3r_linear decoder_embed;
  const d3r_dec_block* dec1;
  const d3r_dec_block* dec2;
  d3r_norm dec_norm;
  const d3r_dpt_head* dpt[2];
  d3r_linear lin_head[2];
} d3r_model;

int d3r_sizeof_model(void);

int64_t d3r_forward_workspace_bytes(const d3r_model* m, int32_t n_enc, int32_t B, int32_t H, int32_t W);

int d3r_forward_pairs(const d3r_model* m, const float* imgs_dev, int32_t n_enc, const int32_t* idx1_host,
                      const int32_t* idx2_host, int32_t B, int32_t H, int32_t W, float* pts3d_1, float* conf_1,
                      float* pts3d_2, float* conf_2, void* workspace_dev, int64_t workspace_bytes, void* stream);

int64_t d3r_forward_mixed_workspace_bytes(const d3r_model* m, int32_t B, int32_t H1, int32_t W1, int32_t H2, int32_t W2);
int d3r_forward_pairs_mixed(const d3r_model* m, const float* imgs1_dev, int32_t H1, int32_t W1, const float* imgs2_dev,
                            int32_t H2, int32_t W2, int32_t B, float* pts3d_1, float* conf_1, float* pts3d_2,
                            float* conf_2, void* workspace_dev, int64_t workspace_bytes, void* stream);

int d3r_forward_set_debug(int32_t stage_id, float* out_dev, int64_t capacity_floats);

#ifdef __cplusplus
}
#endif
#endif
```

Before: 170.1.

## Add ping-pong warpgroup GEMM schedule and wide-N conv tiles

Adds a ping-pong GEMM kernel in which two consumer warpgroups alternate whole 128x128 tiles, ordered by named barriers, so one warpgroup's epilogue overlaps the other's MMA main loop. By default it is used for residual-epilogue GEMMs with short K (at most 12 k-blocks). The change also lets 3x3 convs with simple flags use BLOCK_N=256 when there are enough M tiles per SM, and factors the producer, prologue and epilogue into shared device helpers. The cost is more kernel variants and schedule-selection heuristics, and wider conv tiles may hurt occupancy or load balance.

```diff
diff --git a/dust3r_b200/_lib_fwd.py b/dust3r_b200/_lib_fwd.py
--- a/dust3r_b200/_lib_fwd.py
+++ b/dust3r_b200/_lib_fwd.py
@@ -71,6 +71,10 @@
     lib.d3r_set_gemm_impl.argtypes = [i32]
     lib.d3r_set_gemm_store.restype = None
     lib.d3r_set_gemm_store.argtypes = [i32]
+    lib.d3r_set_gemm_schedule.restype = None
+    lib.d3r_set_gemm_schedule.argtypes = [i32]
+    lib.d3r_set_conv_wide_min_tiles_per_sm.restype = None
+    lib.d3r_set_conv_wide_min_tiles_per_sm.argtypes = [i32]
     lib.d3r_set_attention_impl.restype = None
     lib.d3r_set_attention_impl.argtypes = [i32]
     lib.d3r_forward_workspace_bytes.restype = i64
diff --git a/dust3r_b200/csrc/gemm_host.cu b/dust3r_b200/csrc/gemm_host.cu
--- a/dust3r_b200/csrc/gemm_host.cu
+++ b/dust3r_b200/csrc/gemm_host.cu
@@ -5,9 +5,12 @@
 namespace d3r {
 namespace gemm {
 
-static int pick_block_n(int N, int mode, uint32_t flags) {
+static int g_conv_wide_min_per_sm = 4;
+
+static int pick_block_n(int N, int mode, uint32_t flags, int m_tiles) {
   if (flags & F_HEAD_FINAL) return 128;
   if (N % 256 == 0 && pick_epi(mode, flags) != EPI_GENERIC) return 256;
+  if (N % 256 == 0 && mode == 1 && (flags & ~kConvWideFlags) == 0 && m_tiles >= (long long)g_conv_wide_min_per_sm * num_sms()) return 256;
   if (N % 128 == 0) return 128;
   if (N % 64 == 0) return 64;
   return (N > 128) ? 128 : 64;
@@ -19,13 +22,43 @@
 
 static int g_store = 1;
 
-template <int BN, int EPI, bool PAIR, bool TMA_STORE = false>
+static int g_schedule = 1;
+
+static bool use_pingpong(int mode, uint32_t flags, int N, int num_kb) {
+  if (g_schedule == 0 || N % 128 != 0) return false;
+  const int epi = pick_epi(mode, flags);
+  if (mode != 1 && epi == EPI_GENERIC) return false;
+  if (g_schedule == 2) return true;
+  return mode == 0 && epi == EPI_RESID && num_kb <= 12;
+}
+
+template <int BN, int EPI, bool PAIR, bool TMA_STORE, bool PP>
+static auto kernel_fn() {
+  if constexpr (PP) return gemm_pingpong_kernel<EPI, PAIR, TMA_STORE>;
+  else return gemm_kernel<BN, EPI, PAIR, TMA_STORE>;
+}
+
+template <bool PAIR, bool PP>
+static const char* kernel_tag(int BN, const Params& p) {
+  if (p.mode == 1) {
+    if (p.flags & F_HEAD_FINAL)
+      return PP ? (PAIR ? "conv3x3_head_tail_pingpong_2cta" : "conv3x3_head_tail_pingpong") : (PAIR ? "conv3x3_head_tail_2cta" : "conv3x3_head_tail");
+    return PP ? (PAIR ? "conv3x3_pingpong_2cta" : "conv3x3_pingpong") : (PAIR ? "conv3x3_wgmma_2cta" : "conv3x3_wgmma");
+  }
+  if (PP) return PAIR ? "gemm_pingpong_2cta" : "gemm_pingpong";
+  return BN == 256 ? (PAIR ? "gemm_wgmma_2cta_bn256" : "gemm_wgmma_bn256")
+                   : (PAIR ? "gemm_wgmma_2cta_bn128" : (BN == 128 ? "gemm_wgmma_bn128" : "gemm_wgmma_bn64"));
+}
+
+template <int BN, int EPI, bool PAIR, bool TMA_STORE = false, bool PP = false>
 static int launch(const CUtensorMap& ta, const CUtensorMap& tb, const CUtensorMap& to, const Params& p, int m_tiles, int n_tiles,
                   cudaStream_t st) {
+  static_assert(!PP || BN == 128, "ping-pong tiles are 128x128");
   constexpr int kSmem = Cfg<BN, TMA_STORE>::kSmemBytes;
+  const auto kernel = kernel_fn<BN, EPI, PAIR, TMA_STORE, PP>();
   static unsigned long long attr_devices = 0;
   if (first_launch_on_this_device(attr_devices))
-    D3R_CUDA(cudaFuncSetAttribute(gemm_kernel<BN, EPI, PAIR, TMA_STORE>, cudaFuncAttributeMaxDynamicSharedMemorySize, kSmem));
+    D3R_CUDA(cudaFuncSetAttribute(kernel, cudaFuncAttributeMaxDynamicSharedMemorySize, kSmem));
   int grid;
   if (PAIR) {
     const int items = ((m_tiles + 1) / 2) * n_tiles;
@@ -35,46 +68,42 @@
     const int items = m_tiles * n_tiles;
     grid = items < num_sms() ? items : num_sms();
   }
-  const char* tag = (p.mode == 1) ? ((p.flags & F_HEAD_FINAL) ? (PAIR ? "conv3x3_head_tail_2cta" : "conv3x3_head_tail")
-                                                              : (PAIR ? "conv3x3_wgmma_2cta" : "conv3x3_wgmma"))
-                                  : (BN == 256 ? (PAIR ? "gemm_wgmma_2cta_bn256" : "gemm_wgmma_bn256")
-                                               : (PAIR ? "gemm_wgmma_2cta_bn128" : (BN == 128 ? "gemm_wgmma_bn128" : "gemm_wgmma_bn64")));
   char detail[96];
   snprintf(detail, sizeof(detail), "M=%d N=%d K=%d flags=0x%x mode=%d epi=%d", p.M, p.N, p.K, (unsigned)p.flags, p.mode, EPI);
-  prof::Scope scope(tag, st, 2.0 * double(p.M) * double(p.N) * double(p.K), 0.0, 1, detail);
-  D3R_CUDA(pdl::launch_clustered(gemm_kernel<BN, EPI, PAIR, TMA_STORE>, dim3(grid), dim3(kNumThreads), size_t(kSmem), st, PAIR ? 2 : 1,
-                                 ta, tb, to, p));
+  prof::Scope scope(kernel_tag<PAIR, PP>(BN, p), st, 2.0 * double(p.M) * double(p.N) * double(p.K), 0.0, 1, detail);
+  D3R_CUDA(pdl::launch_clustered(kernel, dim3(grid), dim3(kNumThreads), size_t(kSmem), st, PAIR ? 2 : 1, ta, tb, to, p));
   D3R_LAUNCH_CHECK();
   return D3R_OK;
 }
 
-template <int BN, bool PAIR>
+template <int BN, bool PAIR, bool PP = false>
 static int dispatch_epi(int epi, const CUtensorMap& ta, const CUtensorMap& tb, const CUtensorMap* to, const Params& p, int m_tiles,
                         int n_tiles, cudaStream_t st) {
-  if constexpr (BN == 256) {
+  if constexpr (BN == 256 || PP) {
     if (to) {
       switch (epi) {
-        case EPI_RESID: return launch<BN, EPI_RESID, PAIR, true>(ta, tb, *to, p, m_tiles, n_tiles, st);
-        case EPI_ACT: return launch<BN, EPI_ACT, PAIR, true>(ta, tb, *to, p, m_tiles, n_tiles, st);
-        case EPI_ROPE: return launch<BN, EPI_ROPE, PAIR, true>(ta, tb, *to, p, m_tiles, n_tiles, st);
+        case EPI_RESID: return launch<BN, EPI_RESID, PAIR, true, PP>(ta, tb, *to, p, m_tiles, n_tiles, st);
+        case EPI_ACT: return launch<BN, EPI_ACT, PAIR, true, PP>(ta, tb, *to, p, m_tiles, n_tiles, st);
+        case EPI_ROPE: return launch<BN, EPI_ROPE, PAIR, true, PP>(ta, tb, *to, p, m_tiles, n_tiles, st);
       }
     }
   }
   switch (epi) {
-    case EPI_RESID: return launch<BN, EPI_RESID, PAIR>(ta, tb, tb, p, m_tiles, n_tiles, st);
-    case EPI_ACT: return launch<BN, EPI_ACT, PAIR>(ta, tb, tb, p, m_tiles, n_tiles, st);
-    case EPI_ROPE: return launch<BN, EPI_ROPE, PAIR>(ta, tb, tb, p, m_tiles, n_tiles, st);
-  }
-  if constexpr (BN == 128) return launch<128, EPI_GENERIC, PAIR>(ta, tb, tb, p, m_tiles, n_tiles, st);
+    case EPI_RESID: return launch<BN, EPI_RESID, PAIR, false, PP>(ta, tb, tb, p, m_tiles, n_tiles, st);
+    case EPI_ACT: return launch<BN, EPI_ACT, PAIR, false, PP>(ta, tb, tb, p, m_tiles, n_tiles, st);
+    case EPI_ROPE: return launch<BN, EPI_ROPE, PAIR, false, PP>(ta, tb, tb, p, m_tiles, n_tiles, st);
+  }
+  if constexpr (BN >= 128) return launch<BN, EPI_GENERIC, PAIR, false, PP>(ta, tb, tb, p, m_tiles, n_tiles, st);
   set_error("no BLOCK_N %d kernel for the generic epilogue", BN);
   return D3R_ERR_INVALID;
 }
 
-static int dispatch(int bn, const CUtensorMap& ta, const CUtensorMap& tb, const CUtensorMap* to, const Params& p, int m_tiles,
+static int dispatch(int bn, bool pp, const CUtensorMap& ta, const CUtensorMap& tb, const CUtensorMap* to, const Params& p, int m_tiles,
                     cudaStream_t st) {
   const int n_tiles = (p.N + bn - 1) / bn;
   const int epi = (bn >= 128) ? pick_epi(p.mode, p.flags) : EPI_GENERIC;
   const bool pair = use_pair(bn, p.num_kb);
+  if (pp) return pair ? dispatch_epi<128, true, true>(epi, ta, tb, to, p, m_tiles, n_tiles, st) : dispatch_epi<128, false, true>(epi, ta, tb, to, p, m_tiles, n_tiles, st);
   switch (bn) {
     case 256: return pair ? dispatch_epi<256, true>(epi, ta, tb, to, p, m_tiles, n_tiles, st) : dispatch_epi<256, false>(epi, ta, tb, to, p, m_tiles, n_tiles, st);
     case 128: return pair ? dispatch_epi<128, true>(epi, ta, tb, nullptr, p, m_tiles, n_tiles, st) : dispatch_epi<128, false>(epi, ta, tb, nullptr, p, m_tiles, n_tiles, st);
@@ -99,7 +128,8 @@
   D3R_CHECK_ARG((reinterpret_cast<uintptr_t>(A) & 15) == 0 && (reinterpret_cast<uintptr_t>(B) & 15) == 0, "gemm: operands must be 16-byte aligned");
   p.mode = 0;
   p.num_kb = (p.K + BLOCK_K - 1) / BLOCK_K;
-  const int bn = pick_block_n(p.N, p.mode, p.flags);
+  const bool pp = use_pingpong(p.mode, p.flags, p.N, p.num_kb);
+  const int bn = pp ? 128 : pick_block_n(p.N, p.mode, p.flags, (p.M + BLOCK_M - 1) / BLOCK_M);
   CUtensorMap ta, tb;
   {
     cuuint64_t dims[2] = {(cuuint64_t)p.K, (cuuint64_t)p.M};
@@ -113,7 +143,7 @@
   CUtensorMap to;
   const bool f32 = (p.flags & F_RESID_INPLACE) != 0;
   const long long row_bytes = p.ldo * (f32 ? 4 : 2);
-  const bool staged = g_store == 1 && bn == 256 && pick_epi(p.mode, p.flags) != EPI_GENERIC && p.ldo >= p.N && row_bytes % 16 == 0 &&
+  const bool staged = g_store == 1 && (bn == 256 || pp) && pick_epi(p.mode, p.flags) != EPI_GENERIC && p.ldo >= p.N && row_bytes % 16 == 0 &&
                       (reinterpret_cast<uintptr_t>(p.out) & 15) == 0;
   if (staged) {
     cuuint64_t dims[2] = {(cuuint64_t)p.N, (cuuint64_t)p.M};
@@ -122,7 +152,7 @@
     rc = encode_tensor_map(&to, p.out, 2, dims, str, box, "gemm output", f32 ? CU_TENSOR_MAP_DATA_TYPE_FLOAT32 : CU_TENSOR_MAP_DATA_TYPE_BFLOAT16);
     if (rc) return rc;
   }
-  return dispatch(bn, ta, tb, staged ? &to : nullptr, p, (p.M + BLOCK_M - 1) / BLOCK_M, st);
+  return dispatch(bn, pp, ta, tb, staged ? &to : nullptr, p, (p.M + BLOCK_M - 1) / BLOCK_M, st);
 }
 
 int conv3x3_bf16(const void* x_nhwc, const void* w_packed, int B, int H, int W, int Cin, int Cout, Params p, cudaStream_t st) {
@@ -142,7 +172,8 @@
   p.tiles_x = (W + p.tile_w - 1) / p.tile_w;
   p.tiles_y = (H + p.tile_h - 1) / p.tile_h;
   p.ldo = Cout;
-  const int bn = pick_block_n(p.N, p.mode, p.flags);
+  const bool pp = use_pingpong(p.mode, p.flags, p.N, p.num_kb);
+  const int bn = pp ? 128 : pick_block_n(p.N, p.mode, p.flags, B * p.tiles_x * p.tiles_y);
   CUtensorMap ta, tb;
   {
     cuuint64_t dims[4] = {(cuuint64_t)Cin, (cuuint64_t)W, (cuuint64_t)H, (cuuint64_t)B};
@@ -153,7 +184,7 @@
   }
   int rc = make_tmap_b(&tb, w_packed, Cout, 9, Cin, bn, p.num_kb, "conv3x3");
   if (rc) return rc;
-  return dispatch(bn, ta, tb, nullptr, p, B * p.tiles_x * p.tiles_y, st);
+  return dispatch(bn, pp, ta, tb, nullptr, p, B * p.tiles_x * p.tiles_y, st);
 }
 
 int conv_transpose_bf16(const void* x_nhwc, const void* w_packed, void* out, const float* bias, int B, int h, int w, int Cin, int Cout,
@@ -197,6 +228,8 @@
 extern "C" void d3r_set_gemm_impl(int32_t impl) { gemm::g_impl = impl; }
 extern "C" void d3r_set_gemm_pair_min_kblocks(int32_t kb) { gemm::g_pair_min_kb = kb; }
 extern "C" void d3r_set_gemm_store(int32_t store) { gemm::g_store = store; }
+extern "C" void d3r_set_gemm_schedule(int32_t schedule) { gemm::g_schedule = schedule; }
+extern "C" void d3r_set_conv_wide_min_tiles_per_sm(int32_t tiles) { gemm::g_conv_wide_min_per_sm = tiles; }
 
 extern "C" int d3r_gemm_bf16(const void* A, const void* B, void* out, const float* bias, const void* add0, void* out2,
                              int32_t M, int32_t N, int32_t K, int64_t ldo, uint32_t flags, const float* rope_cos,
diff --git a/dust3r_b200/csrc/gemm_wgmma.cuh b/dust3r_b200/csrc/gemm_wgmma.cuh
--- a/dust3r_b200/csrc/gemm_wgmma.cuh
+++ b/dust3r_b200/csrc/gemm_wgmma.cuh
@@ -57,6 +57,7 @@
 template <> struct EpiMask<EPI_RESID> { static constexpr uint32_t value = F_BIAS | F_RESID_INPLACE; };
 template <> struct EpiMask<EPI_ACT> { static constexpr uint32_t value = F_BIAS | F_GELU | F_RELU; };
 template <> struct EpiMask<EPI_ROPE> { static constexpr uint32_t value = F_BIAS | F_ROPE; };
+constexpr uint32_t kConvWideFlags = F_BIAS | F_RELU | F_ADD0 | F_ADD1 | F_OUT2_RELU;
 __host__ __device__ inline int pick_epi(int mode, uint32_t flags) {
   if (mode != 0) return EPI_GENERIC;
   if ((flags & ~F_BIAS) == F_RESID_INPLACE) return EPI_RESID;
@@ -65,13 +66,13 @@
   return EPI_GENERIC;
 }
 
+constexpr int kOutBuf = 64 * 128;
 template <int BLOCK_N, bool TMA_STORE = false>
 struct Cfg {
   static constexpr int kStageA = BLOCK_M * BLOCK_K * 2;
   static constexpr int kStageB = BLOCK_N * BLOCK_K * 2;
   static constexpr int kStages = (BLOCK_N == 256) ? 4 : (BLOCK_N == 128) ? 6 : 8;
   static constexpr int kRing = kStages * (kStageA + kStageB);
-  static constexpr int kOutBuf = 64 * 128;
   static constexpr int kStaging = TMA_STORE ? 2 * 2 * kOutBuf : 0;
   static constexpr int kSmemBytes = kRing + kStaging + 1024  + 256  + (TMA_STORE ? 0 : (4 * 128 + 16) * 4) ;
   static_assert(kSmemBytes <= 227 * 1024, "shared memory of one CTA");
@@ -91,6 +92,287 @@
   return fmaxf(x, 0.f) - fabsf(h);
 }
 
+template <class C>
+struct Smem {
+  uint8_t* a;
+  uint8_t* b;
+  uint8_t* o;
+  uint64_t* full_bar;
+  uint64_t* empty_bar;
+  float* w4;
+  __device__ __forceinline__ explicit Smem(uint8_t* raw) {
+    uint8_t* s = reinterpret_cast<uint8_t*>((reinterpret_cast<uintptr_t>(raw) + 1023) & ~uintptr_t(1023));
+    a = s;
+    b = s + C::kStages * C::kStageA;
+    o = s + C::kRing;
+    full_bar = reinterpret_cast<uint64_t*>(s + C::kRing + C::kStaging);
+    empty_bar = full_bar + C::kStages;
+    w4 = reinterpret_cast<float*>(reinterpret_cast<uint8_t*>(full_bar) + 256);
+  }
+};
+
+template <class C, bool PAIR, bool TMA_STORE>
+__device__ __forceinline__ void prologue(const Smem<C>& sm, const CUtensorMap* tmap_a, const CUtensorMap* tmap_b,
+                                         const CUtensorMap* tmap_o, const Params& p, uint32_t empty_count) {
+  if (threadIdx.x == 0) {
+    ptx::prefetch_tmap(tmap_a);
+    ptx::prefetch_tmap(tmap_b);
+    if constexpr (TMA_STORE) ptx::prefetch_tmap(tmap_o);
+    for (int s = 0; s < C::kStages; ++s) {
+      ptx::mbar_init(ptx::smem_u32(&sm.full_bar[s]), 1);
+      ptx::mbar_init(ptx::smem_u32(&sm.empty_bar[s]), empty_count);
+    }
+    ptx::fence_barrier_init();
+  }
+  if (!TMA_STORE && (p.flags & F_HEAD_FINAL) && threadIdx.x >= 128) {
+    for (int i = threadIdx.x - 128; i < 4 * 128 + 4; i += 256) sm.w4[i] = (i < 512) ? p.w4[i] : p.b4[i - 512];
+  }
+  __syncthreads();
+  if constexpr (PAIR) ptx::cluster_sync();
+  pdl::sync_with_predecessor();
+}
+
+template <int BLOCK_N, bool PAIR, class C>
+__device__ __forceinline__ void produce(const Smem<C>& sm, const CUtensorMap* tmap_a, const CUtensorMap* tmap_b, const Params& p,
+                                        uint32_t rank, int first_item, int total_items, int item_stride, int n_tiles) {
+  int stage = 0;
+  uint32_t phase = 0;
+  for (int item = first_item; item < total_items; item += item_stride) {
+    const int tn = item % n_tiles, tm = (item / n_tiles) * (PAIR ? 2 : 1) + int(rank);
+    int cb = 0, cy0 = 0, cx0 = 0;
+    if (p.mode == 1) {
+      cb = tm / (p.tiles_y * p.tiles_x);
+      const int r = tm - cb * (p.tiles_y * p.tiles_x);
+      cy0 = (r / p.tiles_x) * p.tile_h;
+      cx0 = (r % p.tiles_x) * p.tile_w;
+    }
+    for (int kb = 0; kb < p.num_kb; ++kb) {
+      ptx::mbar_wait(ptx::smem_u32(&sm.empty_bar[stage]), phase ^ 1);
+      const uint32_t fb = ptx::smem_u32(&sm.full_bar[stage]);
+      ptx::mbar_arrive_expect_tx(fb, C::kStageA + C::kStageB);
+      const uint32_t sa = ptx::smem_u32(sm.a + stage * C::kStageA);
+      const uint32_t sb = ptx::smem_u32(sm.b + stage * C::kStageB);
+      int ka, kt = 0;
+      if (p.mode == 1) {
+        const int tap = kb / p.cin_blocks, cblk = kb - tap * p.cin_blocks;
+        const int dy = tap / 3, dx = tap - dy * 3;
+        ptx::tma_load_4d(sa, tmap_a, fb, cblk * BLOCK_K, cx0 + dx - 1, cy0 + dy - 1, cb);
+        ka = cblk * BLOCK_K;
+        kt = tap;
+      } else {
+        ptx::tma_load_2d(sa, tmap_a, fb, kb * BLOCK_K, tm * BLOCK_M);
+        ka = kb * BLOCK_K;
+      }
+      if constexpr (PAIR) {
+        constexpr int kHalf = BLOCK_N / 2;
+        ptx::tma_load_3d_mc(sb + rank * (kHalf * BLOCK_K * 2), tmap_b, fb, ka, kt, tn * BLOCK_N + int(rank) * kHalf, 0x3);
+      } else {
+        ptx::tma_load_3d(sb, tmap_b, fb, ka, kt, tn * BLOCK_N);
+      }
+      if (++stage == C::kStages) { stage = 0; phase ^= 1; }
+    }
+  }
+}
+
+template <bool PAIR>
+__device__ __forceinline__ void release_slot(uint64_t* empty_bar, int s) {
+  if ((threadIdx.x & 31) == 0) {
+    if constexpr (PAIR) {
+      ptx::mbar_arrive_cluster(ptx::smem_u32(&empty_bar[s]), 0);
+      ptx::mbar_arrive_cluster(ptx::smem_u32(&empty_bar[s]), 1);
+    } else {
+      ptx::mbar_arrive(ptx::smem_u32(&empty_bar[s]));
+    }
+  }
+}
+
+template <int BLOCK_N, int EPI, bool TMA_STORE>
+__device__ __forceinline__ void epilogue_half(float (&acc)[BLOCK_N / 2], const Params& p, const CUtensorMap* tmap_o, int tm, int tn,
+                                              int m_tiles, int row_base, uint8_t* stage_o, uint32_t& out_chunk, uint32_t bar_id,
+                                              const float* s_w4) {
+  const int lane = threadIdx.x & 31, wq = (threadIdx.x >> 5) & 3, q = lane & 3;
+  const uint32_t flags = p.flags & ((EPI == EPI_GENERIC && BLOCK_N == 256) ? kConvWideFlags : EpiMask<EPI>::value);
+  constexpr int kNB = BLOCK_N / 8;
+  bool valid[2];
+  long long row_off[2];
+  int tok[2] = {0, 0};
+  long long pix[2] = {0, 0};
+  int ct_b[2] = {0, 0}, ct_iy[2] = {0, 0}, ct_ix[2] = {0, 0};
+#pragma unroll
+  for (int h = 0; h < 2; ++h) {
+    const int row_in_tile = row_base + wq * 16 + (lane >> 2) + 8 * h;
+    if (p.mode == 1) {
+      const int cb = tm / (p.tiles_y * p.tiles_x);
+      const int r = tm - cb * (p.tiles_y * p.tiles_x);
+      const int y = (r / p.tiles_x) * p.tile_h + row_in_tile / p.tile_w;
+      const int x = (r % p.tiles_x) * p.tile_w + row_in_tile % p.tile_w;
+      valid[h] = (tm < m_tiles) && (y < p.cH) && (x < p.cW);
+      pix[h] = (long long)(cb * p.cH + y) * p.cW + x;
+      row_off[h] = pix[h] * p.ldo;
+    } else {
+      const int row = tm * BLOCK_M + row_in_tile;
+      valid[h] = row < p.M;
+      row_off[h] = (long long)row * p.ldo;
+      if (flags & F_ROPE) tok[h] = row % p.tokens_per_img;
+      if (flags & F_CONVT) {
+        ct_b[h] = row / (p.th_in * p.tw_in);
+        const int r = row - ct_b[h] * (p.th_in * p.tw_in);
+        ct_iy[h] = r / p.tw_in;
+        ct_ix[h] = r - ct_iy[h] * p.tw_in;
+      }
+    }
+  }
+  if (flags & (F_BIAS | F_GELU)) {
+#pragma unroll
+    for (int j = 0; j < kNB; ++j) {
+      const int c = tn * BLOCK_N + 8 * j + 2 * q;
+      float2 b = make_float2(0.f, 0.f);
+      if ((flags & F_BIAS) && c < p.N) {
+        if (flags & F_CONVT) b = make_float2(__ldg(p.bias + c % p.tCout), __ldg(p.bias + (c + 1) % p.tCout));
+        else b = __ldg(reinterpret_cast<const float2*>(p.bias + c));
+      }
+#pragma unroll
+      for (int h = 0; h < 2; ++h) {
+        float& v0 = acc[4 * j + 2 * h];
+        float& v1 = acc[4 * j + 2 * h + 1];
+        v0 += b.x;
+        v1 += b.y;
+        if (flags & F_GELU) { v0 = gelu_erf(v0); v1 = gelu_erf(v1); }
+      }
+    }
+  }
+  if (flags & F_ROPE) {
+#pragma unroll
+    for (int cb = 0; cb < BLOCK_N / 32; ++cb) {
+      const int col0 = tn * BLOCK_N + cb * 32;
+      if (col0 >= p.rope_cols) continue;
+#pragma unroll
+      for (int h = 0; h < 2; ++h) {
+        const int pos = ((col0 & 63) < 32) ? (tok[h] / p.grid_w) : (tok[h] % p.grid_w);
+#pragma unroll
+        for (int jj = 0; jj < 2; ++jj) {
+          const int k = 8 * jj + 2 * q;
+          const float2 cs = __ldg(reinterpret_cast<const float2*>(p.rope_cos + pos * 16 + k));
+          const float2 sn = __ldg(reinterpret_cast<const float2*>(p.rope_sin + pos * 16 + k));
+          const float cc[2] = {cs.x, cs.y}, ss[2] = {sn.x, sn.y};
+#pragma unroll
+          for (int e = 0; e < 2; ++e) {
+            float& u = acc[(4 * cb + jj) * 4 + 2 * h + e];
+            float& w = acc[(4 * cb + jj + 2) * 4 + 2 * h + e];
+            const float u0 = u, w0 = w;
+            u = u0 * cc[e] - w0 * ss[e];
+            w = w0 * cc[e] + u0 * ss[e];
+          }
+        }
+      }
+    }
+  }
+  if constexpr (TMA_STORE) {
+    constexpr bool kF32 = (EPI == EPI_RESID);
+    constexpr int kChunkCols = kF32 ? 32 : 64;
+    constexpr int kChunkNB = kChunkCols / 8;
+    const bool issuer = (threadIdx.x & 127) == 0;
+    const uint32_t sw = lane >> 2;
+#pragma unroll
+    for (int c = 0; c < BLOCK_N / kChunkCols; ++c) {
+      const uint32_t buf = ptx::smem_u32(stage_o + (out_chunk & 1) * kOutBuf);
+#pragma unroll
+      for (int j = 0; j < kChunkNB; ++j)
+#pragma unroll
+        for (int h = 0; h < 2; ++h) {
+          const uint32_t row = wq * 16 + (lane >> 2) + 8 * h;
+          float v0 = acc[4 * (c * kChunkNB + j) + 2 * h], v1 = acc[4 * (c * kChunkNB + j) + 2 * h + 1];
+          if (flags & F_RELU) { v0 = fmaxf(v0, 0.f); v1 = fmaxf(v1, 0.f); }
+          if constexpr (kF32) {
+            ptx::st_shared_v2_f32(buf + row * 128 + (((2 * j + (q >> 1)) ^ sw) << 4) + (q & 1) * 8, v0, v1);
+          } else {
+            ptx::st_shared_b32(buf + row * 128 + ((j ^ sw) << 4) + q * 4, pack_bf16x2(v0, v1));
+          }
+        }
+      ptx::fence_proxy_async();
+      if (issuer) ptx::bulk_wait_group_read<0>();
+      ptx::named_bar_sync(bar_id, 128);
+      if (issuer) {
+        const int c0 = tn * BLOCK_N + c * kChunkCols, r0 = tm * BLOCK_M + row_base;
+        if constexpr (kF32) ptx::tma_reduce_add_2d(tmap_o, buf, c0, r0);
+        else ptx::tma_store_2d(tmap_o, buf, c0, r0);
+        ptx::bulk_commit_group();
+      }
+      ++out_chunk;
+    }
+    return;
+  }
+  if (flags & F_HEAD_FINAL) {
+    float head_acc[2][4] = {{0.f, 0.f, 0.f, 0.f}, {0.f, 0.f, 0.f, 0.f}};
+#pragma unroll
+    for (int j = 0; j < kNB; ++j)
+#pragma unroll
+      for (int h = 0; h < 2; ++h)
+#pragma unroll
+        for (int e = 0; e < 2; ++e) {
+          const float r = fmaxf(acc[4 * j + 2 * h + e], 0.f);
+          const int c = 8 * j + 2 * q + e;
+#pragma unroll
+          for (int o = 0; o < 4; ++o) head_acc[h][o] += r * s_w4[o * 128 + c];
+        }
+#pragma unroll
+    for (int h = 0; h < 2; ++h)
+#pragma unroll
+      for (int o = 0; o < 4; ++o) {
+        head_acc[h][o] += __shfl_xor_sync(0xffffffffu, head_acc[h][o], 1);
+        head_acc[h][o] += __shfl_xor_sync(0xffffffffu, head_acc[h][o], 2);
+      }
+#pragma unroll
+    for (int h = 0; h < 2; ++h) {
+      if (!valid[h] || q != 0) continue;
+      postprocess_pixel(head_acc[h][0] + s_w4[512 + 0], head_acc[h][1] + s_w4[512 + 1], head_acc[h][2] + s_w4[512 + 2],
+                        [&] { return head_acc[h][3] + s_w4[512 + 3]; }, p.pts3d, p.conf, pix[h], p.depth_mode, p.conf_mode,
+                        p.conf_min, p.conf_max);
+    }
+    return;
+  }
+#pragma unroll
+  for (int h = 0; h < 2; ++h) {
+    if (!valid[h]) continue;
+#pragma unroll
+    for (int j = 0; j < kNB; ++j) {
+      const int col = tn * BLOCK_N + 8 * j + 2 * q;
+      if (col >= p.N) continue;
+      float v0 = acc[4 * j + 2 * h], v1 = acc[4 * j + 2 * h + 1];
+      long long off;
+      if (flags & F_CONVT) {
+        const int kk = col / p.tCout, co = col - kk * p.tCout;
+        const int ky = kk / p.tk, kx = kk - ky * p.tk;
+        off = ((long long)(ct_b[h] * p.th_in * p.tk + ct_iy[h] * p.tk + ky) * (p.tw_in * p.tk) + ct_ix[h] * p.tk + kx) * p.tCout + co;
+      } else {
+        off = row_off[h] + col;
+      }
+      if (flags & F_ADD0) {
+        const float2 a = bf16x2_to_float2(__ldg(reinterpret_cast<const unsigned int*>(reinterpret_cast<const __nv_bfloat16*>(p.add0) + off)));
+        v0 += a.x; v1 += a.y;
+      }
+      if (flags & F_ADD1) {
+        const float2 a = bf16x2_to_float2(__ldg(reinterpret_cast<const unsigned int*>(reinterpret_cast<const __nv_bfloat16*>(p.add1) + off)));
+        v0 += a.x; v1 += a.y;
+      }
+      if (flags & F_RELU) { v0 = fmaxf(v0, 0.f); v1 = fmaxf(v1, 0.f); }
+      if (flags & (F_OUT_F32 | F_RESID_INPLACE)) {
+        float2* o = reinterpret_cast<float2*>(reinterpret_cast<float*>(p.out) + off);
+        if (flags & F_RESID_INPLACE) {
+          const float2 r = *o;
+          v0 += r.x; v1 += r.y;
+        }
+        *o = make_float2(v0, v1);
+        if (flags & F_OUT2_BF16) *reinterpret_cast<uint32_t*>(reinterpret_cast<__nv_bfloat16*>(p.out2) + off) = pack_bf16x2(v0, v1);
+      } else {
+        *reinterpret_cast<uint32_t*>(reinterpret_cast<__nv_bfloat16*>(p.out) + off) = pack_bf16x2(v0, v1);
+        if (flags & F_OUT2_RELU)
+          *reinterpret_cast<uint32_t*>(reinterpret_cast<__nv_bfloat16*>(p.out2) + off) = pack_bf16x2(fmaxf(v0, 0.f), fmaxf(v1, 0.f));
+      }
+    }
+  }
+}
+
 template <int BLOCK_N, int EPI, bool PAIR, bool TMA_STORE>
 __global__ void __launch_bounds__(kNumThreads, 1)
 gemm_kernel(const __grid_constant__ CUtensorMap tmap_a, const __grid_constant__ CUtensorMap tmap_b,
@@ -98,16 +380,9 @@
   static_assert(!TMA_STORE || (BLOCK_N == 256 && EPI != EPI_GENERIC), "TMA-store epilogue: specialised epilogues on 128x256 tiles");
   using C = Cfg<BLOCK_N, TMA_STORE>;
   extern __shared__ uint8_t smem_raw[];
-  uint8_t* smem = reinterpret_cast<uint8_t*>((reinterpret_cast<uintptr_t>(smem_raw) + 1023) & ~uintptr_t(1023));
-  uint8_t* smem_a = smem;
-  uint8_t* smem_b = smem + C::kStages * C::kStageA;
-  uint8_t* smem_o = smem + C::kRing;
-  uint64_t* bars = reinterpret_cast<uint64_t*>(smem + C::kRing + C::kStaging);
-  uint64_t* full_bar = bars;
-  uint64_t* empty_bar = bars + C::kStages;
-  float* s_w4 = reinterpret_cast<float*>(reinterpret_cast<uint8_t*>(bars) + 256);
-
-  const int warp = threadIdx.x >> 5, lane = threadIdx.x & 31;
+  const Smem<C> sm(smem_raw);
+
+  const int warp = threadIdx.x >> 5;
   const uint32_t rank = PAIR ? ptx::cluster_ctarank() : 0u;
   const int n_tiles = (p.N + BLOCK_N - 1) / BLOCK_N;
   const int m_tiles = (p.mode == 1) ? p.cB * p.tiles_y * p.tiles_x : (p.M + BLOCK_M - 1) / BLOCK_M;
@@ -116,92 +391,25 @@
   const int first_item = PAIR ? blockIdx.x / 2 : blockIdx.x;
   const int item_stride = PAIR ? gridDim.x / 2 : gridDim.x;
 
-  if (threadIdx.x == 0) {
-    ptx::prefetch_tmap(&tmap_a);
-    ptx::prefetch_tmap(&tmap_b);
-    if constexpr (TMA_STORE) ptx::prefetch_tmap(&tmap_o);
-    for (int s = 0; s < C::kStages; ++s) {
-      ptx::mbar_init(ptx::smem_u32(&full_bar[s]), 1);
-      ptx::mbar_init(ptx::smem_u32(&empty_bar[s]), (PAIR ? 2 : 1) * kConsumerWarps);
-    }
-    ptx::fence_barrier_init();
-  }
-  if (!TMA_STORE && (p.flags & F_HEAD_FINAL) && threadIdx.x >= 128) {
-    for (int i = threadIdx.x - 128; i < 4 * 128 + 4; i += 256) s_w4[i] = (i < 512) ? p.w4[i] : p.b4[i - 512];
-  }
-  __syncthreads();
-  if constexpr (PAIR) ptx::cluster_sync();
-  pdl::sync_with_predecessor();
+  prologue<C, PAIR, TMA_STORE>(sm, &tmap_a, &tmap_b, &tmap_o, p, (PAIR ? 2 : 1) * kConsumerWarps);
 
   if (warp < 4) {
     ptx::setmaxnreg_dec<40>();
-    if (warp == 0 && ptx::elect_one()) {
-      int stage = 0;
-      uint32_t phase = 0;
-      for (int item = first_item; item < total_items; item += item_stride) {
-        const int tn = item % n_tiles, tm = (item / n_tiles) * (PAIR ? 2 : 1) + int(rank);
-        int cb = 0, cy0 = 0, cx0 = 0;
-        if (p.mode == 1) {
-          cb = tm / (p.tiles_y * p.tiles_x);
-          const int r = tm - cb * (p.tiles_y * p.tiles_x);
-          cy0 = (r / p.tiles_x) * p.tile_h;
-          cx0 = (r % p.tiles_x) * p.tile_w;
-        }
-        for (int kb = 0; kb < p.num_kb; ++kb) {
-          ptx::mbar_wait(ptx::smem_u32(&empty_bar[stage]), phase ^ 1);
-          const uint32_t fb = ptx::smem_u32(&full_bar[stage]);
-          ptx::mbar_arrive_expect_tx(fb, C::kStageA + C::kStageB);
-          const uint32_t sa = ptx::smem_u32(smem_a + stage * C::kStageA);
-          const uint32_t sb = ptx::smem_u32(smem_b + stage * C::kStageB);
-          int ka, kt = 0;
-          if (p.mode == 1) {
-            const int tap = kb / p.cin_blocks, cblk = kb - tap * p.cin_blocks;
-            const int dy = tap / 3, dx = tap - dy * 3;
-            ptx::tma_load_4d(sa, &tmap_a, fb, cblk * BLOCK_K, cx0 + dx - 1, cy0 + dy - 1, cb);
-            ka = cblk * BLOCK_K;
-            kt = tap;
-          } else {
-            ptx::tma_load_2d(sa, &tmap_a, fb, kb * BLOCK_K, tm * BLOCK_M);
-            ka = kb * BLOCK_K;
-          }
-          if constexpr (PAIR) {
-            constexpr int kHalf = BLOCK_N / 2;
-            ptx::tma_load_3d_mc(sb + rank * (kHalf * BLOCK_K * 2), &tmap_b, fb, ka, kt, tn * BLOCK_N + int(rank) * kHalf, 0x3);
-          } else {
-            ptx::tma_load_3d(sb, &tmap_b, fb, ka, kt, tn * BLOCK_N);
-          }
-          if (++stage == C::kStages) { stage = 0; phase ^= 1; }
-        }
-      }
-    }
+    if (warp == 0 && ptx::elect_one()) produce<BLOCK_N, PAIR>(sm, &tmap_a, &tmap_b, p, rank, first_item, total_items, item_stride, n_tiles);
   } else {
     ptx::setmaxnreg_inc<232>();
     const int wg = (threadIdx.x >> 7) - 1;
-    const int wq = warp & 3;
-    const int q = lane & 3;
-    const uint32_t flags = p.flags & EpiMask<EPI>::value;
-    constexpr int kNB = BLOCK_N / 8;
     float acc[BLOCK_N / 2];
     int stage = 0;
     uint32_t phase = 0;
     uint32_t out_chunk = 0;
-    auto release = [&](int s) {
-      if (lane == 0) {
-        if constexpr (PAIR) {
-          ptx::mbar_arrive_cluster(ptx::smem_u32(&empty_bar[s]), 0);
-          ptx::mbar_arrive_cluster(ptx::smem_u32(&empty_bar[s]), 1);
-        } else {
-          ptx::mbar_arrive(ptx::smem_u32(&empty_bar[s]));
-        }
-      }
-    };
     for (int item = first_item; item < total_items; item += item_stride) {
       const int tn = item % n_tiles, tm = (item / n_tiles) * (PAIR ? 2 : 1) + int(rank);
       int prev = -1;
       for (int kb = 0; kb < p.num_kb; ++kb) {
-        ptx::mbar_wait(ptx::smem_u32(&full_bar[stage]), phase);
-        const uint64_t da = ptx::desc_kmajor_sw128(ptx::smem_u32(smem_a + stage * C::kStageA + wg * 64 * 128));
-        const uint64_t db = ptx::desc_kmajor_sw128(ptx::smem_u32(smem_b + stage * C::kStageB));
+        ptx::mbar_wait(ptx::smem_u32(&sm.full_bar[stage]), phase);
+        const uint64_t da = ptx::desc_kmajor_sw128(ptx::smem_u32(sm.a + stage * C::kStageA + wg * 64 * 128));
+        const uint64_t db = ptx::desc_kmajor_sw128(ptx::smem_u32(sm.b + stage * C::kStageB));
         ptx::wgmma_fence();
 #pragma unroll
         for (int k = 0; k < BLOCK_K / WGMMA_K; ++k) {
@@ -211,192 +419,14 @@
         }
         ptx::wgmma_commit();
         ptx::wgmma_wait<1>();
-        if (prev >= 0) release(prev);
+        if (prev >= 0) release_slot<PAIR>(sm.empty_bar, prev);
         prev = stage;
         if (++stage == C::kStages) { stage = 0; phase ^= 1; }
       }
       ptx::wgmma_wait<0>();
       ptx::reg_fence(acc);
-      release(prev);
-
-      bool valid[2];
-      long long row_off[2];
-      int tok[2] = {0, 0};
-      long long pix[2] = {0, 0};
-      int ct_b[2] = {0, 0}, ct_iy[2] = {0, 0}, ct_ix[2] = {0, 0};
-#pragma unroll
-      for (int h = 0; h < 2; ++h) {
-        const int row_in_tile = wg * 64 + wq * 16 + (lane >> 2) + 8 * h;
-        if (p.mode == 1) {
-          const int cb = tm / (p.tiles_y * p.tiles_x);
-          const int r = tm - cb * (p.tiles_y * p.tiles_x);
-          const int y = (r / p.tiles_x) * p.tile_h + row_in_tile / p.tile_w;
-          const int x = (r % p.tiles_x) * p.tile_w + row_in_tile % p.tile_w;
-          valid[h] = (tm < m_tiles) && (y < p.cH) && (x < p.cW);
-          pix[h] = (long long)(cb * p.cH + y) * p.cW + x;
-          row_off[h] = pix[h] * p.ldo;
-        } else {
-          const int row = tm * BLOCK_M + row_in_tile;
-          valid[h] = row < p.M;
-          row_off[h] = (long long)row * p.ldo;
-          if (flags & F_ROPE) tok[h] = row % p.tokens_per_img;
-          if (flags & F_CONVT) {
-            ct_b[h] = row / (p.th_in * p.tw_in);
-            const int r = row - ct_b[h] * (p.th_in * p.tw_in);
-            ct_iy[h] = r / p.tw_in;
-            ct_ix[h] = r - ct_iy[h] * p.tw_in;
-          }
-        }
-      }
-      if (flags & (F_BIAS | F_GELU)) {
-#pragma unroll
-        for (int j = 0; j < kNB; ++j) {
-          const int c = tn * BLOCK_N + 8 * j + 2 * q;
-          float2 b = make_float2(0.f, 0.f);
-          if ((flags & F_BIAS) && c < p.N) {
-            if (flags & F_CONVT) b = make_float2(__ldg(p.bias + c % p.tCout), __ldg(p.bias + (c + 1) % p.tCout));
-            else b = __ldg(reinterpret_cast<const float2*>(p.bias + c));
-          }
-#pragma unroll
-          for (int h = 0; h < 2; ++h) {
-            float& v0 = acc[4 * j + 2 * h];
-            float& v1 = acc[4 * j + 2 * h + 1];
-            v0 += b.x;
-            v1 += b.y;
-            if (flags & F_GELU) { v0 = gelu_erf(v0); v1 = gelu_erf(v1); }
-          }
-        }
-      }
-      if (flags & F_ROPE) {
-#pragma unroll
-        for (int cb = 0; cb < BLOCK_N / 32; ++cb) {
-          const int col0 = tn * BLOCK_N + cb * 32;
-          if (col0 >= p.rope_cols) continue;
-#pragma unroll
-          for (int h = 0; h < 2; ++h) {
-            const int pos = ((col0 & 63) < 32) ? (tok[h] / p.grid_w) : (tok[h] % p.grid_w);
-#pragma unroll
-            for (int jj = 0; jj < 2; ++jj) {
-              const int k = 8 * jj + 2 * q;
-              const float2 cs = __ldg(reinterpret_cast<const float2*>(p.rope_cos + pos * 16 + k));
-              const float2 sn = __ldg(reinterpret_cast<const float2*>(p.rope_sin + pos * 16 + k));
-              const float cc[2] = {cs.x, cs.y}, ss[2] = {sn.x, sn.y};
-#pragma unroll
-              for (int e = 0; e < 2; ++e) {
-                float& u = acc[(4 * cb + jj) * 4 + 2 * h + e];
-                float& w = acc[(4 * cb + jj + 2) * 4 + 2 * h + e];
-                const float u0 = u, w0 = w;
-                u = u0 * cc[e] - w0 * ss[e];
-                w = w0 * cc[e] + u0 * ss[e];
-              }
-            }
-          }
-        }
-      }
-      if constexpr (TMA_STORE) {
-        constexpr bool kF32 = (EPI == EPI_RESID);
-        constexpr int kChunkCols = kF32 ? 32 : 64;
-        constexpr int kChunkNB = kChunkCols / 8;
-        const bool issuer = (threadIdx.x & 127) == 0;
-        const uint32_t sw = lane >> 2;
-#pragma unroll
-        for (int c = 0; c < BLOCK_N / kChunkCols; ++c) {
-          const uint32_t buf = ptx::smem_u32(smem_o + (wg * 2 + (out_chunk & 1)) * C::kOutBuf);
-#pragma unroll
-          for (int j = 0; j < kChunkNB; ++j)
-#pragma unroll
-            for (int h = 0; h < 2; ++h) {
-              const uint32_t row = wq * 16 + (lane >> 2) + 8 * h;
-              float v0 = acc[4 * (c * kChunkNB + j) + 2 * h], v1 = acc[4 * (c * kChunkNB + j) + 2 * h + 1];
-              if (flags & F_RELU) { v0 = fmaxf(v0, 0.f); v1 = fmaxf(v1, 0.f); }
-              if constexpr (kF32) {
-                ptx::st_shared_v2_f32(buf + row * 128 + (((2 * j + (q >> 1)) ^ sw) << 4) + (q & 1) * 8, v0, v1);
-              } else {
-                ptx::st_shared_b32(buf + row * 128 + ((j ^ sw) << 4) + q * 4, pack_bf16x2(v0, v1));
-              }
-            }
-          ptx::fence_proxy_async();
-          if (issuer) ptx::bulk_wait_group_read<0>();
-          ptx::named_bar_sync(1 + wg, 128);
-          if (issuer) {
-            const int c0 = tn * BLOCK_N + c * kChunkCols, r0 = tm * BLOCK_M + wg * 64;
-            if constexpr (kF32) ptx::tma_reduce_add_2d(&tmap_o, buf, c0, r0);
-            else ptx::tma_store_2d(&tmap_o, buf, c0, r0);
-            ptx::bulk_commit_group();
-          }
-          ++out_chunk;
-        }
-        continue;
-      }
-      if (flags & F_HEAD_FINAL) {
-        float head_acc[2][4] = {{0.f, 0.f, 0.f, 0.f}, {0.f, 0.f, 0.f, 0.f}};
-#pragma unroll
-        for (int j = 0; j < kNB; ++j)
-#pragma unroll
-          for (int h = 0; h < 2; ++h)
-#pragma unroll
-            for (int e = 0; e < 2; ++e) {
-              const float r = fmaxf(acc[4 * j + 2 * h + e], 0.f);
-              const int c = 8 * j + 2 * q + e;
-#pragma unroll
-              for (int o = 0; o < 4; ++o) head_acc[h][o] += r * s_w4[o * 128 + c];
-            }
-#pragma unroll
-        for (int h = 0; h < 2; ++h)
-#pragma unroll
-          for (int o = 0; o < 4; ++o) {
-            head_acc[h][o] += __shfl_xor_sync(0xffffffffu, head_acc[h][o], 1);
-            head_acc[h][o] += __shfl_xor_sync(0xffffffffu, head_acc[h][o], 2);
-          }
-#pragma unroll
-        for (int h = 0; h < 2; ++h) {
-          if (!valid[h] || q != 0) continue;
-          postprocess_pixel(head_acc[h][0] + s_w4[512 + 0], head_acc[h][1] + s_w4[512 + 1], head_acc[h][2] + s_w4[512 + 2],
-                            [&] { return head_acc[h][3] + s_w4[512 + 3]; }, p.pts3d, p.conf, pix[h], p.depth_mode, p.conf_mode,
-                            p.conf_min, p.conf_max);
-        }
-        continue;
-      }
-#pragma unroll
-      for (int h = 0; h < 2; ++h) {
-        if (!valid[h]) continue;
-#pragma unroll
-        for (int j = 0; j < kNB; ++j) {
-          const int col = tn * BLOCK_N + 8 * j + 2 * q;
-          if (col >= p.N) continue;
-          float v0 = acc[4 * j + 2 * h], v1 = acc[4 * j + 2 * h + 1];
-          long long off;
-          if (flags & F_CONVT) {
-            const int kk = col / p.tCout, co = col - kk * p.tCout;
-            const int ky = kk / p.tk, kx = kk - ky * p.tk;
-            off = ((long long)(ct_b[h] * p.th_in * p.tk + ct_iy[h] * p.tk + ky) * (p.tw_in * p.tk) + ct_ix[h] * p.tk + kx) * p.tCout + co;
-          } else {
-            off = row_off[h] + col;
-          }
-          if (flags & F_ADD0) {
-            const float2 a = bf16x2_to_float2(__ldg(reinterpret_cast<const unsigned int*>(reinterpret_cast<const __nv_bfloat16*>(p.add0) + off)));
-            v0 += a.x; v1 += a.y;
-          }
-          if (flags & F_ADD1) {
-            const float2 a = bf16x2_to_float2(__ldg(reinterpret_cast<const unsigned int*>(reinterpret_cast<const __nv_bfloat16*>(p.add1) + off)));
-            v0 += a.x; v1 += a.y;
-          }
-          if (flags & F_RELU) { v0 = fmaxf(v0, 0.f); v1 = fmaxf(v1, 0.f); }
-          if (flags & (F_OUT_F32 | F_RESID_INPLACE)) {
-            float2* o = reinterpret_cast<float2*>(reinterpret_cast<float*>(p.out) + off);
-            if (flags & F_RESID_INPLACE) {
-              const float2 r = *o;
-              v0 += r.x; v1 += r.y;
-            }
-            *o = make_float2(v0, v1);
-            if (flags & F_OUT2_BF16) *reinterpret_cast<uint32_t*>(reinterpret_cast<__nv_bfloat16*>(p.out2) + off) = pack_bf16x2(v0, v1);
-          } else {
-            *reinterpret_cast<uint32_t*>(reinterpret_cast<__nv_bfloat16*>(p.out) + off) = pack_bf16x2(v0, v1);
-            if (flags & F_OUT2_RELU)
-              *reinterpret_cast<uint32_t*>(reinterpret_cast<__nv_bfloat16*>(p.out2) + off) = pack_bf16x2(fmaxf(v0, 0.f), fmaxf(v1, 0.f));
-          }
-        }
-      }
+      release_slot<PAIR>(sm.empty_bar, prev);
+      epilogue_half<BLOCK_N, EPI, TMA_STORE>(acc, p, &tmap_o, tm, tn, m_tiles, wg * 64, sm.o + wg * 2 * kOutBuf, out_chunk, 1 + wg, sm.w4);
     }
     if constexpr (TMA_STORE) {
       if ((threadIdx.x & 127) == 0) ptx::bulk_wait_group<0>();
@@ -405,5 +435,83 @@
   if constexpr (PAIR) ptx::cluster_sync();
 }
 
-}
-}
+template <int EPI, bool PAIR, bool TMA_STORE>
+__global__ void __launch_bounds__(kNumThreads, 1)
+gemm_pingpong_kernel(const __grid_constant__ CUtensorMap tmap_a, const __grid_constant__ CUtensorMap tmap_b,
+                     const __grid_constant__ CUtensorMap tmap_o, const Params p) {
+  static_assert(!TMA_STORE || EPI != EPI_GENERIC, "TMA-store epilogue: specialised epilogues");
+  constexpr int BLOCK_N = 128;
+  constexpr uint32_t kOrderBar = 3;
+  using C = Cfg<BLOCK_N, TMA_STORE>;
+  extern __shared__ uint8_t smem_raw[];
+  const Smem<C> sm(smem_raw);
+
+  const int warp = threadIdx.x >> 5;
+  const uint32_t rank = PAIR ? ptx::cluster_ctarank() : 0u;
+  const int n_tiles = p.N / BLOCK_N;
+  const int m_tiles = (p.mode == 1) ? p.cB * p.tiles_y * p.tiles_x : (p.M + BLOCK_M - 1) / BLOCK_M;
+  const int m_groups = PAIR ? (m_tiles + 1) / 2 : m_tiles;
+  const int total_items = m_groups * n_tiles;
+  const int first_item = PAIR ? blockIdx.x / 2 : blockIdx.x;
+  const int item_stride = PAIR ? gridDim.x / 2 : gridDim.x;
+
+  prologue<C, PAIR, TMA_STORE>(sm, &tmap_a, &tmap_b, &tmap_o, p, (PAIR ? 2 : 1) * 4);
+
+  if (warp < 4) {
+    ptx::setmaxnreg_dec<40>();
+    if (warp == 0 && ptx::elect_one()) produce<BLOCK_N, PAIR>(sm, &tmap_a, &tmap_b, p, rank, first_item, total_items, item_stride, n_tiles);
+  } else {
+    ptx::setmaxnreg_inc<232>();
+    const int wg = (threadIdx.x >> 7) - 1;
+    float acc[2][BLOCK_N / 2];
+    int stage = 0;
+    uint32_t phase = 0;
+    uint32_t out_chunk = 0;
+    int local = 0;
+    for (int item = first_item; item < total_items; item += item_stride, ++local) {
+      if ((local & 1) != wg) {
+        stage += p.num_kb;
+        phase ^= uint32_t(stage / C::kStages) & 1u;
+        stage %= C::kStages;
+        continue;
+      }
+      const int tn = item % n_tiles, tm = (item / n_tiles) * (PAIR ? 2 : 1) + int(rank);
+      if (local > 0) ptx::named_bar_sync(kOrderBar + wg, 256);
+      int prev = -1;
+      for (int kb = 0; kb < p.num_kb; ++kb) {
+        ptx::mbar_wait(ptx::smem_u32(&sm.full_bar[stage]), phase);
+        const uint32_t sa = ptx::smem_u32(sm.a + stage * C::kStageA);
+        const uint64_t da0 = ptx::desc_kmajor_sw128(sa);
+        const uint64_t da1 = ptx::desc_kmajor_sw128(sa + 64 * 128);
+        const uint64_t db = ptx::desc_kmajor_sw128(ptx::smem_u32(sm.b + stage * C::kStageB));
+        ptx::wgmma_fence();
+#pragma unroll
+        for (int k = 0; k < BLOCK_K / WGMMA_K; ++k) {
+          const uint32_t accumulate = (kb | k) != 0 ? 1u : 0u;
+          ptx::wgmma_m64n128k16_ss(acc[0], da0 + uint64_t(2 * k), db + uint64_t(2 * k), accumulate);
+          ptx::wgmma_m64n128k16_ss(acc[1], da1 + uint64_t(2 * k), db + uint64_t(2 * k), accumulate);
+        }
+        ptx::wgmma_commit();
+        ptx::wgmma_wait<1>();
+        if (prev >= 0) release_slot<PAIR>(sm.empty_bar, prev);
+        prev = stage;
+        if (++stage == C::kStages) { stage = 0; phase ^= 1; }
+      }
+      if (item + item_stride < total_items) ptx::named_bar_arrive(kOrderBar + (wg ^ 1), 256);
+      ptx::wgmma_wait<0>();
+      ptx::reg_fence(acc[0]);
+      ptx::reg_fence(acc[1]);
+      release_slot<PAIR>(sm.empty_bar, prev);
+      uint8_t* stage_o = sm.o + wg * 2 * kOutBuf;
+      epilogue_half<BLOCK_N, EPI, TMA_STORE>(acc[0], p, &tmap_o, tm, tn, m_tiles, 0, stage_o, out_chunk, 1 + wg, sm.w4);
+      epilogue_half<BLOCK_N, EPI, TMA_STORE>(acc[1], p, &tmap_o, tm, tn, m_tiles, 64, stage_o, out_chunk, 1 + wg, sm.w4);
+    }
+    if constexpr (TMA_STORE) {
+      if ((threadIdx.x & 127) == 0) ptx::bulk_wait_group<0>();
+    }
+  }
+  if constexpr (PAIR) ptx::cluster_sync();
+}
+
+}
+}
diff --git a/dust3r_b200/csrc/sm90_ptx.cuh b/dust3r_b200/csrc/sm90_ptx.cuh
--- a/dust3r_b200/csrc/sm90_ptx.cuh
+++ b/dust3r_b200/csrc/sm90_ptx.cuh
@@ -119,6 +119,7 @@
   asm volatile("st.shared.v2.f32 [%0], {%1, %2};" ::"r"(addr), "f"(a), "f"(b) : "memory");
 }
 __device__ __forceinline__ void named_bar_sync(uint32_t id, uint32_t count) { asm volatile("bar.sync %0, %1;" ::"r"(id), "r"(count) : "memory"); }
+__device__ __forceinline__ void named_bar_arrive(uint32_t id, uint32_t count) { asm volatile("bar.arrive %0, %1;" ::"r"(id), "r"(count) : "memory"); }
 
 __device__ __forceinline__ uint32_t cluster_ctarank() {
   uint32_t r;
diff --git a/include/dust3r_b200.h b/include/dust3r_b200.h
--- a/include/dust3r_b200.h
+++ b/include/dust3r_b200.h
@@ -166,6 +166,8 @@
 void d3r_set_gemm_impl(int32_t impl);
 void d3r_set_gemm_pair_min_kblocks(int32_t kblocks);
 void d3r_set_gemm_store(int32_t store);
+void d3r_set_gemm_schedule(int32_t schedule);
+void d3r_set_conv_wide_min_tiles_per_sm(int32_t tiles);
 
 void d3r_set_attention_impl(int32_t impl);
 
```

After: 174.9 (median of 6 runs). +2.9%, better.
